# cmavro/GNN-RAG

Measured on AMD Instinct MI355X. Metric: kg_edges_aggregated_per_sec, higher is better.
Workload: dtype f32

## Files before the change

### gnn-rag_amd/csrc/dense_internal.h

```cpp
#pragma once
#include "gnnrag_common.h"

namespace gnnrag {

int tables_vq_launch_z(const gnnrag_csr* csr, const void* planes, const float* ins, const float* W, float* P, int32_t D,
                       int32_t I, int32_t only_dir, float* zero, int64_t zero_n, hipStream_t stream);

int update_b3_launch_z(const float* h, const float* nbr, const float* W, const float* b, const float* w_s,
                       const float* b_s, const float* mask, float* h_out, float* score, int64_t BN, int32_t D,
                       int32_t ldw, hipStream_t stream, bool score_zeroed);

int update_score_fused_rows(const float* h, const float* nbr, const uint8_t* add_flag, const float* W, const float* b,
                            const float* w_s, const float* b_s, const float* mask, float* h_out, float* score,
                            int64_t BN, int32_t D, int32_t I, int32_t math, hipStream_t stream, bool score_zeroed);
int update_b3_launch_f(const float* h, const float* nbr, const uint8_t* add_flag, const float* W, const float* b,
                       const float* w_s, const float* b_s, const float* mask, float* h_out, float* score, int64_t BN,
                       int32_t D, int32_t ldw, hipStream_t stream, bool score_zeroed);

bool update_rows_supported(const float* h, const float* nbr, const float* W, const float* h_out, int64_t BN, int32_t D,
                           int32_t I, int32_t math);
bool update_b3_shape_ok(int64_t BN, int32_t D, int32_t ldw);
int tables_small_launch(const gnnrag_csr* csr, const float* T_fwd, const float* T_inv, const float* ins, const float* W,
                        float* P, int32_t D, int32_t I, hipStream_t stream);

int frontier_build_z(const gnnrag_csr* csr, const float* dist, void* fws, size_t fws_bytes, float* zero_a,
                     int64_t zero_na, float* zero_b, int64_t zero_nb, hipStream_t stream);
const uint8_t* frontier_row_flags(const gnnrag_csr* csr, const void* fws);

int update_score_fused_z(const float* h, const float* nbr, const float* W, const float* b, const float* w_s,
                         const float* b_s, const float* mask, float* h_out, float* score, int64_t BN, int32_t D,
                         int32_t I, int32_t math, hipStream_t stream, bool score_zeroed);

bool rel_transform_accepts(const float* relfeat_fwd, const float* relfeat_inv, int64_t R1, int32_t D, int32_t L,
                           const gnnrag_layer_params* layers, int32_t pos_rows, const float* T_out, const void* planes_out);

}
```

### gnn-rag_amd/csrc/frontier.hip

```cpp
#include "dense_internal.h"

namespace gnnrag {

constexpr int kFrThreads = 1024;
constexpr int kFrSeedCap = 2048;
constexpr int kFrAltSeeds = 32;

struct FrontierWs {
  size_t counts, row_flag, rows, tflag, trows, seeds, seedinfo, total;
};

static FrontierWs frontier_ws(const gnnrag_csr* csr) {
  FrontierWs w;
  size_t off = 0;
  auto take = [&](size_t bytes) { size_t o = off; off = align_up(off + bytes, 256); return o; };
  const size_t BN = (size_t)csr->B * csr->N;
  const size_t RT = (size_t)(csr->rel_total > 0 ? csr->rel_total : 1);
  w.counts = take((size_t)2 * csr->B * sizeof(int32_t));
  w.row_flag = take(BN + 64);
  w.rows = take(BN * sizeof(int32_t));
  w.tflag = take(RT + 64);
  w.trows = take(RT * sizeof(int32_t));
  w.seeds = take((size_t)csr->B * kFrAltSeeds * sizeof(int32_t));
  w.seedinfo = take((size_t)2 * csr->B * sizeof(int32_t));
  w.total = off;
  return w;
}

__global__ __launch_bounds__(kFrThreads) void k_frontier_build(
    const float* __restrict__ dist, const int32_t* __restrict__ rp0, const int32_t* __restrict__ rp1,
    const int2* __restrict__ el0, const int2* __restrict__ el1, const int32_t* __restrict__ rel_off, int N,
    uint8_t* __restrict__ row_flag, int32_t* __restrict__ rows, uint8_t* __restrict__ tflag,
    int32_t* __restrict__ trows, int32_t* __restrict__ counts, int32_t* __restrict__ seeds,
    int32_t* __restrict__ seedinfo, float* __restrict__ zero_a, long long zero_na, float* __restrict__ zero_b,
    long long zero_nb) {
  __shared__ int s_seed[kFrSeedCap];
  __shared__ int s_ns, s_wsum[kFrThreads / 64];
  const int g = blockIdx.x, tid = threadIdx.x, lane = tid & 63, wave = tid >> 6;
  const int roff = rel_off[g], Rg = rel_off[g + 1] - roff;
  const size_t n0 = (size_t)g * N;
  for (long long i = (long long)blockIdx.x * kFrThreads + tid; i < zero_na; i += (long long)gridDim.x * kFrThreads) zero_a[i] = 0.f;
  for (long long i = (long long)blockIdx.x * kFrThreads + tid; i < zero_nb; i += (long long)gridDim.x * kFrThreads) zero_b[i] = 0.f;
  if (tid == 0) s_ns = 0;
  if (g == (int)gridDim.x - 1 && tid < 64) row_flag[(size_t)gridDim.x * N + tid] = 0;
  for (int i = tid; i < N; i += kFrThreads) row_flag[n0 + i] = 0;
  for (int i = tid; i < Rg; i += kFrThreads) tflag[roff + i] = 0;
  __syncthreads();
  for (int i = tid; i < N; i += kFrThreads) {
    if (dist[n0 + i] != 0.f) {
      const int k = atomicAdd(&s_ns, 1);
      if (k < kFrSeedCap) s_seed[k] = (int)n0 + i;
    }
  }
  __syncthreads();
  const int ns = s_ns;
  if (tid == 0) {
    int cnt = -1, facts = 0;
    if (ns <= kFrAltSeeds) {
      cnt = ns;
      for (int i = 1; i < ns; ++i) {
        const int v = s_seed[i];
        int j = i - 1;
        for (; j >= 0 && s_seed[j] > v; --j) s_seed[j + 1] = s_seed[j];
        s_seed[j + 1] = v;
      }
      for (int i = 0; i < ns; ++i) {
        const int sn = s_seed[i];
        seeds[g * kFrAltSeeds + i] = sn;
        facts += (rp0[sn + 1] - rp0[sn]) + (rp1[sn + 1] - rp1[sn]);
      }
    }
    seedinfo[2 * g] = cnt;
    seedinfo[2 * g + 1] = facts;
  }
  __syncthreads();
  if (ns > kFrSeedCap) {
    for (int i = tid; i < N; i += kFrThreads) row_flag[n0 + i] = 1;
    for (int i = tid; i < Rg; i += kFrThreads) tflag[roff + i] = 1;
  } else {
    for (int k = 0; k < ns; ++k) {
      const int s = s_seed[k];
#pragma unroll
      for (int dd = 0; dd < 2; ++dd) {
        const int32_t* rp = dd ? rp1 : rp0;
        const int2* el = dd ? el1 : el0;
        const int beg = rp[s], end = rp[s + 1];
        for (int j = beg + tid; j < end; j += kFrThreads) {
          const int2 e = el[j];
          row_flag[e.x] = 1;
          tflag[roff + e.y] = 1;
        }
      }
    }
  }
  __syncthreads();
  auto compact = [&](const uint8_t* flag, int n, int first, int32_t* list, int32_t* count_out) {
    int base = 0;
    for (int c0 = 0; c0 < n; c0 += kFrThreads) {
      const int i = c0 + tid;
      const bool on = i < n && flag[i] != 0;
      const unsigned long long m = __ballot(on);
      if (lane == 0) s_wsum[wave] = __popcll(m);
      __syncthreads();
      int off = base, tot = 0;
      for (int w = 0; w < kFrThreads / 64; ++w) {
        const int c = s_wsum[w];
        if (w < wave) off += c;
        tot += c;
      }
      if (on) list[off + __popcll(m & ((1ull << lane) - 1))] = first + i;
      base += tot;
      __syncthreads();
    }
    if (tid == 0) *count_out = base;
  };
  compact(row_flag + n0, N, (int)n0, rows + n0, counts + 2 * g);
  compact(tflag + roff, Rg, roff, trows + roff, counts + 2 * g + 1);
}

struct TabFrArgs {
  const float* T[2];
  const float* ins;
  const float* W;
  const int2* rel_rows;
  const int32_t* rel_off;
  const int32_t* list;
  const int32_t* counts;
  float* P;
  int32_t D, I, rel_total, B;
  int32_t dense;
};

__global__ __launch_bounds__(256) void k_tables_frontier(TabFrArgs a, int tiles_per_q) {
  __shared__ __attribute__((aligned(16))) float s_part[3][4][64][4];
  const int lane = threadIdx.x & 63, wave = threadIdx.x >> 6;
  const int fr = lane & 15, fg = lane >> 4;
  const int D = a.D, K = a.I * D, ldw = (2 * a.I + 1) * D;
  const int ncg = (D + 63) >> 6;
  const f32x4 zero4 = {0.f, 0.f, 0.f, 0.f};
  const int nitem = a.dense ? ((a.rel_total + 15) >> 4) * 2 * ncg : a.B * 2 * ncg;
  for (int item = blockIdx.x; item < nitem; item += gridDim.x)
  for (int tile = a.dense ? item / (2 * ncg) : 0; tile < (a.dense ? item / (2 * ncg) + 1 : tiles_per_q); ++tile) {
    int r = a.dense ? item % (2 * ncg) : item;
    const int cg = r % ncg; r /= ncg;
    const int d = r & 1; r >>= 1;
    const int g = a.dense ? 0 : r;
    const int cnt = a.dense ? a.rel_total : a.counts[2 * g + 1];
    if (tile * 16 >= cnt) break;
    const int32_t* list = a.dense ? nullptr : a.list + a.rel_off[g];
    const int c0 = cg * 64;
    const int m = tile * 16 + fr;
    const int prow = a.dense ? (m < cnt ? m : cnt - 1) : list[m < cnt ? m : cnt - 1];
    const int2 br = a.rel_rows[prow];
    const float* trow = a.T[d] + (size_t)br.y * D;
    const float* qrow = a.ins + (size_t)br.x * a.I * D;
    const float* wrow[4];
#pragma unroll
    for (int nt = 0; nt < 4; ++nt) wrow[nt] = a.W + (size_t)min(c0 + nt * 16 + fr, D - 1) * ldw + (size_t)(1 + d) * D;
    f32x4 acc[4] = {zero4, zero4, zero4, zero4};
    const int nkg = (K + 15) >> 4;
    for (int kg0 = wave; kg0 < nkg; kg0 += 16) {
      f32x4 av[4], bv[4][4];
#pragma unroll
      for (int u = 0; u < 4; ++u) {
        const int k = (kg0 + 4 * u) * 16 + fg * 4;
        av[u] = zero4;
#pragma unroll
        for (int nt = 0; nt < 4; ++nt) bv[u][nt] = zero4;
        if (k < K) {
          const int i = k / D, kk = k - i * D;
          const f32x4 t = *reinterpret_cast<const f32x4*>(trow + kk);
          const f32x4 q = *reinterpret_cast<const f32x4*>(qrow + (size_t)i * D + kk);
          av[u] = __builtin_elementwise_max(t * q, zero4);
#pragma unroll
          for (int nt = 0; nt < 4; ++nt) bv[u][nt] = *reinterpret_cast<const f32x4*>(wrow[nt] + (size_t)2 * i * D + kk);
        }
      }
#pragma unroll
      for (int u = 0; u < 4; ++u)
#pragma unroll
        for (int nt = 0; nt < 4; ++nt)
#pragma unroll
          for (int e = 0; e < 4; ++e) acc[nt] = __builtin_amdgcn_mfma_f32_16x16x4f32(av[u][e], bv[u][nt][e], acc[nt], 0, 0, 0);
    }
    if (wave > 0) {
#pragma unroll
      for (int nt = 0; nt < 4; ++nt) *reinterpret_cast<f32x4*>(&s_part[wave - 1][nt][lane][0]) = acc[nt];
    }
    __syncthreads();
    if (wave == 0) {
#pragma unroll
      for (int nt = 0; nt < 4; ++nt) {
        const f32x4 v = ((acc[nt] + *reinterpret_cast<const f32x4*>(&s_part[0][nt][lane][0])) +
                         *reinterpret_cast<const f32x4*>(&s_part[1][nt][lane][0])) +
                        *reinterpret_cast<const f32x4*>(&s_part[2][nt][lane][0]);
        const int col = c0 + nt * 16 + fr;
#pragma unroll
        for (int rr = 0; rr < 4; ++rr) {
          const int mm = tile * 16 + fg * 4 + rr;
          if (mm < cnt && col < D) a.P[((size_t)d * a.rel_total + (a.dense ? mm : list[mm])) * D + col] = v[rr];
        }
      }
    }
    __syncthreads();
  }
}

struct WalkFrArgs {
  const int32_t* rp0;
  const int32_t* rp1;
  const int2* edge_m;
  const int32_t* m_from;
  const float* w0;
  const float* w1;
  const float* dist;
  const float* P;
  const int32_t* rel_off;
  const int32_t* rows;
  const int32_t* counts;
  float* out;
  const int32_t* seeds;
  const int32_t* seedinfo;
  int64_t F;
  int32_t N, D, rel_total, B;
};

constexpr int kWfThreads = 256;
constexpr int kWfPer = 8;
constexpr int kWfCap = kWfThreads * kWfPer;
constexpr int kWfAltMin = 4096;

__global__ __launch_bounds__(kWfThreads) void k_walk_frontier(WalkFrArgs a, int per_q) {
  __shared__ int2 s_live[kWfCap];
  __shared__ int s_wsum[kWfPer * 4];
  __shared__ __attribute__((aligned(16))) float s_red[3][256];
  const int tid = threadIdx.x, lane = tid & 63, wave = tid >> 6;
  const int D = a.D;
  const int g = blockIdx.x / per_q;
  const int cnt = a.counts[2 * g];
  const int roff = a.rel_off[g], Rg = a.rel_off[g + 1] - roff;
  const int col = 4 * lane;
  const bool cok = col < D;
  const f32x4 zero4 = {0.f, 0.f, 0.f, 0.f};
  for (int it = blockIdx.x % per_q; it < cnt; it += per_q) {
    const int n = a.rows[(size_t)g * a.N + it];
    const int beg = a.rp0[n] + a.rp1[n], end = a.rp0[n + 1] + a.rp1[n + 1];
    f32x4 acc = zero4;
    bool split = false;
    const int nseed = a.seedinfo[2 * g];
    const bool alt = nseed > 0 && end - beg > kWfAltMin && a.seedinfo[2 * g + 1] <= ((end - beg) >> 2);
    if (alt && wave == 0) {
      for (int si = 0; si < nseed; ++si) {
        const int sn = a.seeds[g * kFrAltSeeds + si];
        const float ps = a.dist[sn];
        const int sb = a.rp0[sn] + a.rp1[sn], se = a.rp0[sn + 1] + a.rp1[sn + 1];
        for (int c0 = sb; c0 < se; c0 += 64) {
          const int j = c0 + lane;
          const int2 e = j < se ? a.edge_m[j] : make_int2(-1, 0);
          float p = 0.f;
          if (e.x == n) {
            p = ps;
            if (a.w0) {
              const int f = a.m_from[j];
              p *= f < a.F ? a.w0[f] : a.w1[f - a.F];
            }
          }
          unsigned long long m = __ballot(p != 0.f);
          while (m) {
            const int l = __builtin_ctzll(m);
            m &= m - 1;
            const float pl = __int_as_float(__builtin_amdgcn_readlane(__float_as_int(p), l));
            const int rm = __builtin_amdgcn_readlane(e.y, l);
            const int dq = rm > Rg ? 1 : 0;
            const int rl = dq ? rm - (Rg + 1) : rm;
            if (cok) acc += pl * *reinterpret_cast<const f32x4*>(a.P + ((size_t)(1 - dq) * a.rel_total + roff + rl) * D + col);
          }
        }
      }
    }
    for (int c0 = beg; c0 < (alt ? beg : end); c0 += kWfCap) {
      int2 e[kWfPer];
      float p[kWfPer];
#pragma unroll
      for (int u = 0; u < kWfPer; ++u) {
        const int j = c0 + u * kWfThreads + tid;
        e[u] = j < end ? a.edge_m[j] : make_int2(0, 0);
      }
#pragma unroll
      for (int u = 0; u < kWfPer; ++u) {
        const int j = c0 + u * kWfThreads + tid;
        p[u] = 0.f;
        if (j < end) {
          p[u] = a.dist[e[u].x];
          if (a.w0) {
            const int f = a.m_from[j];
            p[u] *= f < a.F ? a.w0[f] : a.w1[f - a.F];
          }
        }
      }
      unsigned long long mk[kWfPer];
#pragma unroll
      for (int u = 0; u < kWfPer; ++u) {
        mk[u] = __ballot(p[u] != 0.f);
        if (lane == 0) s_wsum[u * 4 + wave] = __popcll(mk[u]);
      }
      __syncthreads();
      int nl = 0;
#pragma unroll
      for (int u = 0; u < kWfPer; ++u) {
        int off = nl;
#pragma unroll
        for (int w = 0; w < 4; ++w) {
          const int t = s_wsum[u * 4 + w];
          if (w < wave) off += t;
          nl += t;
        }
        if (p[u] != 0.f) {
          const int rm = e[u].y;
          const int d = rm > Rg ? 1 : 0;
          const int rl = d ? rm - (Rg + 1) : rm;
          s_live[off + __popcll(mk[u] & ((1ull << lane) - 1))] = make_int2(__float_as_int(p[u]), d * a.rel_total + roff + rl);
        }
      }
      __syncthreads();
      if (nl <= 32 && !split) {
        if (wave == 0 && cok) {
          for (int k = 0; k < nl; ++k) {
            const int2 lv = s_live[k];
            const f32x4 t = *reinterpret_cast<const f32x4*>(a.P + (size_t)lv.y * D + col);
            acc += __int_as_float(lv.x) * t;
          }
        }
      } else {
        split = true;
        if (cok) {
          for (int k = wave; k < nl; k += 4) {
            const int2 lv = s_live[k];
            const f32x4 t = *reinterpret_cast<const f32x4*>(a.P + (size_t)lv.y * D + col);
            acc += __int_as_float(lv.x) * t;
          }
        }
      }
      __syncthreads();
    }
    if (split) {
      if (wave > 0) *reinterpret_cast<f32x4*>(&s_red[wave - 1][col]) = acc;
      __syncthreads();
      if (wave == 0)
        acc = ((acc + *reinterpret_cast<const f32x4*>(&s_red[0][col])) + *reinterpret_cast<const f32x4*>(&s_red[1][col])) +
              *reinterpret_cast<const f32x4*>(&s_red[2][col]);
      __syncthreads();
    }
    if (wave == 0 && cok) *reinterpret_cast<f32x4*>(a.out + (size_t)n * D + col) = acc;
  }
}

}

using namespace gnnrag;

extern "C" size_t gnnrag_frontier_workspace_bytes(const gnnrag_csr* csr) {
  if (!csr) return 0;
  return frontier_ws(csr).total;
}

extern "C" int gnnrag_frontier_supported(const gnnrag_csr* csr, int32_t D) {
  return csr && csr->edge_m && csr->m_from && D > 0 && D % 4 == 0 && D <= 256 ? 1 : 0;
}

int gnnrag::frontier_build_z(const gnnrag_csr* csr, const float* dist, void* fws, size_t fws_bytes, float* zero_a,
                             int64_t zero_na, float* zero_b, int64_t zero_nb, hipStream_t stream) {
  if (!csr || !dist || !fws) return GNNRAG_E_BADARG;
  const FrontierWs w = frontier_ws(csr);
  if (fws_bytes < w.total) return GNNRAG_E_WORKSPACE;
  char* base = (char*)fws;
  hipLaunchKernelGGL(k_frontier_build, dim3(csr->B), dim3(kFrThreads), 0, stream, dist, csr->row_ptr[0], csr->row_ptr[1],
                     (const int2*)csr->edge_l[0], (const int2*)csr->edge_l[1], csr->rel_off, csr->N,
                     (uint8_t*)(base + w.row_flag), (int32_t*)(base + w.rows), (uint8_t*)(base + w.tflag),
                     (int32_t*)(base + w.trows), (int32_t*)(base + w.counts), (int32_t*)(base + w.seeds),
                     (int32_t*)(base + w.seedinfo), zero_a, (long long)zero_na, zero_b,
                     (long long)zero_nb);
  GNNRAG_LAUNCH_CHECK();
  return 0;
}

extern "C" int gnnrag_frontier_build(const gnnrag_csr* csr, const float* dist, void* fws, size_t fws_bytes,
                                     gnnrag_stream_t stream) {
  return frontier_build_z(csr, dist, fws, fws_bytes, nullptr, 0, nullptr, 0, (hipStream_t)stream);
}

const uint8_t* gnnrag::frontier_row_flags(const gnnrag_csr* csr, const void* fws) {
  return (const uint8_t*)fws + frontier_ws(csr).row_flag;
}

static bool fr_aligned16(const void* a, const void* b = nullptr, const void* c = nullptr, const void* d = nullptr,
                         const void* e = nullptr) {
  return ((((uintptr_t)a | (uintptr_t)b | (uintptr_t)c | (uintptr_t)d | (uintptr_t)e) & 15) == 0);
}

extern "C" int gnnrag_relation_tables_frontier(const gnnrag_csr* csr, const void* fws, const float* T_fwd,
                                               const float* T_inv, const float* ins, const float* W, float* P,
                                               int32_t D, int32_t I, gnnrag_stream_t stream) {
  if (!csr || !fws || !T_fwd || !T_inv || !ins || !W || !P || I <= 0) return GNNRAG_E_BADARG;
  if (!gnnrag_frontier_supported(csr, D) || !fr_aligned16(T_fwd, T_inv, ins, W, P)) return GNNRAG_E_UNSUPPORTED;
  if (csr->rel_total == 0) return 0;
  const FrontierWs w = frontier_ws(csr);
  const char* base = (const char*)fws;
  TabFrArgs a;
  a.T[0] = T_fwd; a.T[1] = T_inv; a.ins = ins; a.W = W;
  a.rel_rows = (const int2*)csr->rel_rows;
  a.rel_off = csr->rel_off;
  a.list = (const int32_t*)(base + w.trows);
  a.counts = (const int32_t*)(base + w.counts);
  a.P = P; a.D = D; a.I = I; a.rel_total = csr->rel_total; a.B = csr->B; a.dense = 0;
  const int tiles_per_q = (csr->rel_max + 15) / 16;
  const int64_t nitem = (int64_t)csr->B * 2 * ((D + 63) / 64);
  hipLaunchKernelGGL(k_tables_frontier, dim3((unsigned)(nitem < 4096 ? nitem : 4096)), dim3(256), 0, (hipStream_t)stream, a,
                     tiles_per_q);
  GNNRAG_LAUNCH_CHECK();
  return 0;
}

extern "C" int gnnrag_aggregate_fused_frontier(const gnnrag_csr* csr, const void* fws, const float* dist,
                                               const float* P, float* out, int32_t D, gnnrag_stream_t stream) {
  if (!csr || !fws || !dist || !P || !out) return GNNRAG_E_BADARG;
  if (!gnnrag_frontier_supported(csr, D) || !fr_aligned16(P, out) || csr->N <= 0) return GNNRAG_E_UNSUPPORTED;
  const FrontierWs w = frontier_ws(csr);
  const char* base = (const char*)fws;
  WalkFrArgs a;
  a.rp0 = csr->row_ptr[0]; a.rp1 = csr->row_ptr[1];
  a.edge_m = (const int2*)csr->edge_m; a.m_from = csr->m_from;
  a.w0 = csr->w_gnn[0]; a.w1 = csr->w_gnn[1];
  a.dist = dist; a.P = P; a.rel_off = csr->rel_off;
  a.rows = (const int32_t*)(base + w.rows);
  a.counts = (const int32_t*)(base + w.counts);
  a.seeds = (const int32_t*)(base + w.seeds);
  a.seedinfo = (const int32_t*)(base + w.seedinfo);
  a.out = out; a.F = csr->F; a.N = csr->N; a.D = D; a.rel_total = csr->rel_total; a.B = csr->B;
  int per_q = 1024 / csr->B;
  if (per_q < 4) per_q = 4;
  if (per_q > 256) per_q = 256;
  if (per_q > csr->N) per_q = csr->N;
  hipLaunchKernelGGL(k_walk_frontier, dim3((unsigned)(csr->B * per_q)), dim3(kWfThreads), 0, (hipStream_t)stream, a, per_q);
  GNNRAG_LAUNCH_CHECK();
  return 0;
}

extern "C" int gnnrag_frontier_read(const gnnrag_csr* csr, const void* fws, int32_t* counts2, uint8_t* row_flag_host,
                                    gnnrag_stream_t stream) {
  if (!csr || !fws || !counts2) return GNNRAG_E_BADARG;
  const FrontierWs w = frontier_ws(csr);
  const char* base = (const char*)fws;
  int32_t* per_q = new int32_t[(size_t)2 * csr->B];
  hipError_t e = hipMemcpyAsync(per_q, base + w.counts, (size_t)2 * csr->B * sizeof(int32_t), hipMemcpyDeviceToHost,
                                (hipStream_t)stream);
  if (e == hipSuccess && row_flag_host)
    e = hipMemcpyAsync(row_flag_host, base + w.row_flag, (size_t)csr->B * csr->N, hipMemcpyDeviceToHost, (hipStream_t)stream);
  if (e == hipSuccess) e = hipStreamSynchronize((hipStream_t)stream);
  counts2[0] = counts2[1] = 0;
  for (int g = 0; g < csr->B; ++g) {
    counts2[0] += per_q[2 * g];
    counts2[1] += per_q[2 * g + 1];
  }
  delete[] per_q;
  return e == hipSuccess ? 0 : (int)e;
}

int gnnrag::tables_small_launch(const gnnrag_csr* csr, const float* T_fwd, const float* T_inv, const float* ins,
                                const float* W, float* P, int32_t D, int32_t I, hipStream_t stream) {
  if (D % 4 || D > 256 || csr->rel_total <= 0) return GNNRAG_E_UNSUPPORTED;
  if (2.0 * 2 * csr->rel_total * (double)I * D * D > 1.5e8) return GNNRAG_E_UNSUPPORTED;
  if ((((uintptr_t)T_fwd | (uintptr_t)T_inv | (uintptr_t)ins | (uintptr_t)W) & 15) != 0) return GNNRAG_E_UNSUPPORTED;
  TabFrArgs a;
  a.T[0] = T_fwd; a.T[1] = T_inv; a.ins = ins; a.W = W;
  a.rel_rows = (const int2*)csr->rel_rows;
  a.rel_off = csr->rel_off;
  a.list = nullptr; a.counts = nullptr;
  a.P = P; a.D = D; a.I = I; a.rel_total = csr->rel_total; a.B = csr->B; a.dense = 1;
  const int nitem = ((csr->rel_total + 15) / 16) * 2 * ((D + 63) / 64);
  hipLaunchKernelGGL(k_tables_frontier, dim3(nitem), dim3(256), 0, stream, a, 0);
  GNNRAG_LAUNCH_CHECK();
  return 0;
}
```

### gnn-rag_amd/csrc/softmax_layer.hip

```cpp
#include "gnnrag_common.h"
#include "dense_internal.h"

namespace gnnrag {

template <int ITEMS>
__global__ __launch_bounds__(1024) void k_masked_softmax(const float* __restrict__ score,
                                                         float* __restrict__ dist, int N) {
  __shared__ float red[16];
  __shared__ float bcast;
  const float* s = score + (size_t)blockIdx.x * N;
  float* o = dist + (size_t)blockIdx.x * N;
  const int lane = threadIdx.x & 63, wave = threadIdx.x >> 6;
  float v[ITEMS > 0 ? ITEMS : 1];

  float m = -INFINITY;
  if constexpr (ITEMS > 0) {
#pragma unroll
    for (int k = 0; k < ITEMS; ++k) {
      const int i = threadIdx.x + k * 1024;
      v[k] = i < N ? s[i] : -INFINITY;
      m = fmaxf(m, v[k]);
    }
  } else {
    for (int i = threadIdx.x; i < N; i += 1024) m = fmaxf(m, s[i]);
  }
#pragma unroll
  for (int off = 32; off > 0; off >>= 1) m = fmaxf(m, __shfl_xor(m, off, 64));
  if (lane == 0) red[wave] = m;
  __syncthreads();
  if (threadIdx.x == 0) {
    float mm = red[0];
    for (int w = 1; w < 16; ++w) mm = fmaxf(mm, red[w]);
    bcast = mm;
  }
  __syncthreads();
  m = bcast;
  __syncthreads();

  float sum = 0.f;
  if constexpr (ITEMS > 0) {
#pragma unroll
    for (int k = 0; k < ITEMS; ++k) {
      v[k] = expf(v[k] - m);
      sum += v[k];
    }
  } else {
    for (int i = threadIdx.x; i < N; i += 1024) sum += expf(s[i] - m);
  }
#pragma unroll
  for (int off = 32; off > 0; off >>= 1) sum += __shfl_xor(sum, off, 64);
  if (lane == 0) red[wave] = sum;
  __syncthreads();
  if (threadIdx.x == 0) {
    float t = 0.f;
    for (int w = 0; w < 16; ++w) t += red[w];
    bcast = t;
  }
  __syncthreads();
  const float total = bcast;
  if constexpr (ITEMS > 0) {
#pragma unroll
    for (int k = 0; k < ITEMS; ++k) {
      const int i = threadIdx.x + k * 1024;
      if (i < N) o[i] = v[k] / total;
    }
  } else {
    for (int i = threadIdx.x; i < N; i += 1024) o[i] = expf(s[i] - m) / total;
  }
}

template <int ITEMS>
__global__ __launch_bounds__(1024) void k_softmax_pairs(const float* __restrict__ score, float* __restrict__ dist, int N,
                                                        const int32_t* __restrict__ rp0, const int32_t* __restrict__ rp1,
                                                        const int2* __restrict__ em, const int32_t* __restrict__ from,
                                                        const float* __restrict__ w0, const float* __restrict__ w1,
                                                        int64_t F, int2* __restrict__ pr) {
  extern __shared__ float s_dist[];
  __shared__ float red[16];
  __shared__ float bcast;
  const int g = blockIdx.x, part = blockIdx.y, nparts = gridDim.y;
  const float* s = score + (size_t)g * N;
  float* o = dist + (size_t)g * N;
  const int lane = threadIdx.x & 63, wave = threadIdx.x >> 6;
  float v[ITEMS];
  float m = -INFINITY;
#pragma unroll
  for (int k = 0; k < ITEMS; ++k) {
    const int i = threadIdx.x + k * 1024;
    v[k] = i < N ? s[i] : -INFINITY;
    m = fmaxf(m, v[k]);
  }
#pragma unroll
  for (int off = 32; off > 0; off >>= 1) m = fmaxf(m, __shfl_xor(m, off, 64));
  if (lane == 0) red[wave] = m;
  __syncthreads();
  if (threadIdx.x == 0) {
    float mm = red[0];
    for (int w = 1; w < 16; ++w) mm = fmaxf(mm, red[w]);
    bcast = mm;
  }
  __syncthreads();
  m = bcast;
  __syncthreads();
  float sum = 0.f;
#pragma unroll
  for (int k = 0; k < ITEMS; ++k) {
    v[k] = expf(v[k] - m);
    sum += v[k];
  }
#pragma unroll
  for (int off = 32; off > 0; off >>= 1) sum += __shfl_xor(sum, off, 64);
  if (lane == 0) red[wave] = sum;
  __syncthreads();
  if (threadIdx.x == 0) {
    float t = 0.f;
    for (int w = 0; w < 16; ++w) t += red[w];
    bcast = t;
  }
  __syncthreads();
  const float total = bcast;
#pragma unroll
  for (int k = 0; k < ITEMS; ++k) {
    const int i = threadIdx.x + k * 1024;
    if (i < N) {
      const float d = v[k] / total;
      s_dist[i] = d;
      if (part == 0) o[i] = d;
    }
  }
  __syncthreads();
  const int64_t n0 = (int64_t)g * N;
  const int64_t beg = (int64_t)rp0[n0] + rp1[n0], end = (int64_t)rp0[n0 + N] + rp1[n0 + N];
  const int64_t lo = beg + (end - beg) * part / nparts, hi = beg + (end - beg) * (part + 1) / nparts;
  typedef int i32x2 __attribute__((ext_vector_type(2)));
  for (int64_t j = lo + threadIdx.x; j < hi; j += 1024) {
    const i32x2 e = __builtin_nontemporal_load(reinterpret_cast<const i32x2*>(em) + j);
    const unsigned s = (unsigned)(e.x - (int)n0);
    float p = s < (unsigned)N ? s_dist[s] : 0.f;
    if (w0) {
      const int f = from[j];
      p *= f < F ? w0[f] : w1[f - F];
    }
    pr[j] = make_int2(__float_as_int(p), e.y);
  }
}

__global__ __launch_bounds__(256) void k_stream_copy(const f32x4* __restrict__ src, f32x4* __restrict__ dst,
                                                     int64_t n4) {
  const int64_t stride = (int64_t)gridDim.x * 1024;
  for (int64_t base = (int64_t)blockIdx.x * 1024; base < n4; base += stride) {
    f32x4 v[4];
#pragma unroll
    for (int u = 0; u < 4; ++u) {
      const int64_t i = base + u * 256 + threadIdx.x;
      if (i < n4) v[u] = __builtin_nontemporal_load(src + i);
    }
#pragma unroll
    for (int u = 0; u < 4; ++u) {
      const int64_t i = base + u * 256 + threadIdx.x;
      if (i < n4) __builtin_nontemporal_store(v[u], dst + i);
    }
  }
}

struct LayerWs { size_t T_fwd, T_inv, planes, agg, P, nbr, partial, partial_bytes, fws, fws_bytes, total; };

static bool fused_is_cheaper(int64_t B, int64_t N, int64_t rel_total, int64_t D, int64_t I) {
  const double unfused = (double)B * N * (2 * I + 1) * D * D;
  const double fused = 2.0 * rel_total * I * D * D + (double)B * N * D * D;
  return fused < 0.8 * unfused;
}

static bool path_ok(int32_t path) {
  const int base = path & 0xf, flags = path & ~0xf & ~GNNRAG_PATH_SEED_PRIOR & ~GNNRAG_PATH_REUSE_PROJ;
  if (base < GNNRAG_PATH_AUTO || base > GNNRAG_PATH_FUSED) return false;
  return flags == 0 || flags == GNNRAG_PATH_ONLY_FWD || flags == GNNRAG_PATH_ONLY_INV;
}

static LayerWs layer_ws(const gnnrag_csr* csr, int32_t D, int32_t I) {
  LayerWs w;
  size_t off = 0;
  auto take = [&](size_t bytes) { size_t o = off; off = align_up(off + bytes, 256); return o; };
  const size_t BN = (size_t)csr->B * csr->N;
  w.T_fwd = take((size_t)2 * csr->R1 * D * sizeof(float));
  w.T_inv = w.T_fwd + (size_t)csr->R1 * D * sizeof(float);
  w.planes = take(tables_vq_shape_ok(D, I) ? tables_vq_planes_bytes(csr->R1) : 0);
  const size_t a_bytes = BN * 2 * I * D * sizeof(float);
  const size_t p_bytes = align_up((size_t)2 * (csr->rel_total > 0 ? csr->rel_total : 1) * D * sizeof(float), 256);
  const size_t n_bytes = (BN + 1) * D * sizeof(float);
  const size_t big = take(a_bytes > p_bytes + n_bytes ? a_bytes : p_bytes + n_bytes);
  w.agg = big;
  w.P = big;
  w.nbr = big + p_bytes;
  w.partial_bytes = gnnrag_aggregate_workspace_bytes(csr, D, I);
  w.partial = take(w.partial_bytes);
  w.fws_bytes = gnnrag_frontier_workspace_bytes(csr);
  w.fws = take(w.fws_bytes);
  w.total = off;
  return w;
}

static bool planes_wanted(const gnnrag_csr* csr, int32_t D, int32_t I, int32_t path, int32_t math) {
  const bool fused = (path & 0xf) == GNNRAG_PATH_FUSED ||
                     ((path & 0xf) == GNNRAG_PATH_AUTO && fused_is_cheaper(csr->B, csr->N, csr->rel_total, D, I));
  return fused && math != GNNRAG_MATH_FP32 && tables_vq_shape_ok(D, I) && csr->rel_total >= 1024;
}

}

using namespace gnnrag;

extern "C" int gnnrag_masked_softmax(const float* score, float* dist, int32_t B, int32_t N,
                                     gnnrag_stream_t stream) {
  if (!score || !dist || B <= 0 || N <= 0) return GNNRAG_E_BADARG;
  if (N <= 2048) hipLaunchKernelGGL(k_masked_softmax<2>, dim3(B), dim3(1024), 0, (hipStream_t)stream, score, dist, N);
  else if (N <= 8192) hipLaunchKernelGGL(k_masked_softmax<8>, dim3(B), dim3(1024), 0, (hipStream_t)stream, score, dist, N);
  else hipLaunchKernelGGL(k_masked_softmax<0>, dim3(B), dim3(1024), 0, (hipStream_t)stream, score, dist, N);
  GNNRAG_LAUNCH_CHECK();
  return 0;
}

extern "C" int gnnrag_stream_copy(const float* src, float* dst, int64_t n, gnnrag_stream_t stream) {
  if (!src || !dst || n < 0 || (n & 3)) return GNNRAG_E_BADARG;
  if (n == 0) return 0;
  hipLaunchKernelGGL(k_stream_copy, dim3(256 * 16), dim3(256), 0, (hipStream_t)stream, (const f32x4*)src,
                     (f32x4*)dst, n / 4);
  GNNRAG_LAUNCH_CHECK();
  return 0;
}

extern "C" size_t gnnrag_layer_workspace_bytes(const gnnrag_csr* csr, int32_t D, int32_t I) {
  if (!csr || D <= 0 || I <= 0) return 0;
  return layer_ws(csr, D, I).total;
}

static int finish_softmax(const gnnrag_csr* csr, const LayerWs& w, char* base, const float* score, float* dist_out, int32_t D,
                          bool want_pairs, bool* pairs_done, gnnrag_stream_t stream) {
  if (pairs_done) *pairs_done = false;
  const char* env = getenv("GNNRAG_SOFTMAX_PAIRS");
  const bool enabled = !(env && env[0] == '0');
  if (want_pairs && pairs_done && enabled && csr->N <= 8192 && csr->edge_m) {
    PriorPairsTarget t;
    const int rc = prior_pairs_target(csr, D, base + w.partial, w.partial_bytes, &t);
    if (rc) return rc;
    if (t.ok) {
      int parts = (512 + csr->B - 1) / csr->B;
      parts = parts < 1 ? 1 : parts > 8 ? 8 : parts;
      const size_t lds = (size_t)csr->N * sizeof(float);
      if (csr->N <= 2048)
        hipLaunchKernelGGL(k_softmax_pairs<2>, dim3(csr->B, parts), dim3(1024), lds, (hipStream_t)stream, score, dist_out,
                           csr->N, csr->row_ptr[0], csr->row_ptr[1], t.edge_m, t.m_from, t.w0, t.w1, t.F, t.pairs);
      else
        hipLaunchKernelGGL(k_softmax_pairs<8>, dim3(csr->B, parts), dim3(1024), lds, (hipStream_t)stream, score, dist_out,
                           csr->N, csr->row_ptr[0], csr->row_ptr[1], t.edge_m, t.m_from, t.w0, t.w1, t.F, t.pairs);
      GNNRAG_LAUNCH_CHECK();
      *pairs_done = true;
      return 0;
    }
  }
  return gnnrag_masked_softmax(score, dist_out, csr->B, csr->N, stream);
}

static int layer_body(const gnnrag_csr* csr, const LayerWs& w, char* base, const float* h, const float* dist,
                      const float* ins, const float* T_fwd, const float* T_inv, const void* planes, const float* W_e2e,
                      const float* b_e2e, const float* w_score, const float* b_score, const float* mask,
                      float* h_out, float* score_out, float* dist_out, int32_t D, int32_t I, int32_t path,
                      int32_t math, gnnrag_stream_t stream, bool pairs_ready = false, bool* pairs_for_next = nullptr) {
  if (pairs_for_next) *pairs_for_next = false;
  const int64_t BN = (int64_t)csr->B * csr->N;
  int rc;
  const int only = (path & GNNRAG_PATH_ONLY_FWD) ? 0 : (path & GNNRAG_PATH_ONLY_INV) ? 1 : -1;
  const bool seed_prior = (path & GNNRAG_PATH_SEED_PRIOR) != 0;
  path &= 0xf;
  if (path == GNNRAG_PATH_AUTO)
    path = fused_is_cheaper(csr->B, csr->N, csr->rel_total, D, I) ? GNNRAG_PATH_FUSED : GNNRAG_PATH_UNFUSED;
  if (path == GNNRAG_PATH_FUSED) {
    float* P = (float*)(base + w.P);
    float* nbr = (float*)(base + w.nbr);
    const bool one_dir = only >= 0 && gnnrag_aggregate_fused_variant(csr, D) != GNNRAG_WALK_L2_GATHER;
    const bool fr_aligned = ((((uintptr_t)ins | (uintptr_t)W_e2e | (uintptr_t)T_fwd | (uintptr_t)T_inv | (uintptr_t)P |
                               (uintptr_t)nbr | (uintptr_t)dist) & 15) == 0) && csr->N > 0;
    const bool frontier_form = seed_prior && only < 0 && fr_aligned && gnnrag_frontier_supported(csr, D) && csr->rel_total > 0;
    if (frontier_form) {
      void* fws = base + w.fws;
      const bool gated = update_rows_supported(h, nbr, W_e2e, h_out, BN, D, I, math);
      if (!gated) GNNRAG_HIP(hipMemsetAsync(nbr, 0, (size_t)BN * D * sizeof(float), (hipStream_t)stream));
      rc = frontier_build_z(csr, dist, fws, w.fws_bytes, score_out, BN, nbr + (size_t)BN * D, D, (hipStream_t)stream);
      if (rc) return rc;
      rc = gnnrag_relation_tables_frontier(csr, fws, T_fwd, T_inv, ins, W_e2e, P, D, I, stream);
      if (rc) return rc;
      rc = gnnrag_aggregate_fused_frontier(csr, fws, dist, P, nbr, D, stream);
      if (rc) return rc;
      rc = update_score_fused_rows(h, nbr, gated ? frontier_row_flags(csr, fws) : nullptr, W_e2e, b_e2e, w_score, b_score,
                                   mask, h_out, score_out, BN, D, I, math, (hipStream_t)stream, true);
      if (rc) return rc;
      return finish_softmax(csr, w, base, score_out, dist_out, D, only < 0, pairs_for_next, stream);
    }
    rc = GNNRAG_E_UNSUPPORTED;
    bool score_zeroed = false;
    if (planes && math != GNNRAG_MATH_FP32 && csr->rel_total > 0) {
      rc = tables_vq_launch_z(csr, planes, ins, W_e2e, P, D, I, one_dir ? only : -1, score_out, BN, (hipStream_t)stream);
      score_zeroed = rc == 0;
    }
    if (rc == GNNRAG_E_UNSUPPORTED) rc = gnnrag_relation_tables(csr, T_fwd, T_inv, ins, W_e2e, P, D, I, math, stream);
    if (rc) return rc;
    rc = aggregate_fused_dirs(csr, dist, P, nbr, D, one_dir ? 2 - only : 0, base + w.partial, w.partial_bytes,
                              (hipStream_t)stream, pairs_ready && !one_dir);
    if (rc) return rc;
    rc = update_score_fused_z(h, nbr, W_e2e, b_e2e, w_score, b_score, mask, h_out, score_out, BN, D, I, math,
                              (hipStream_t)stream, score_zeroed);
    if (rc) return rc;
    return finish_softmax(csr, w, base, score_out, dist_out, D, only < 0, pairs_for_next, stream);
  } else {
    float* agg = (float*)(base + w.agg);
    rc = gnnrag_aggregate(csr, dist, ins, T_fwd, T_inv, agg, D, I, base + w.partial, w.partial_bytes, stream);
    if (rc) return rc;
    rc = gnnrag_update_score(h, agg, W_e2e, b_e2e, w_score, b_score, mask, h_out, score_out, BN, D, I, math,
                             stream);
    if (rc) return rc;
  }
  return gnnrag_masked_softmax(score_out, dist_out, csr->B, csr->N, stream);
}

static int rel_projections(const gnnrag_csr* csr, int32_t n, const gnnrag_layer_params* layers,
                           const float* relfeat_fwd, const float* relfeat_inv, int32_t pos_rows, float* T,
                           void* planes, bool* planes_written, int32_t D, int32_t math, gnnrag_stream_t stream) {
  *planes_written = false;
  if ((D & 3) == 0) {
    const int rc = gnnrag_rel_transform(relfeat_fwd, relfeat_inv, csr->R1, D, n, layers, pos_rows, T, planes, stream);
    if (rc == 0) *planes_written = planes != nullptr;
    if (rc != GNNRAG_E_UNSUPPORTED) return rc;
  }
  const size_t RD = (size_t)csr->R1 * D;
  for (int j = 0; j < n; ++j) {
    const gnnrag_layer_params& p = layers[j];
    const int rc = gnnrag_linear_pair(relfeat_fwd, relfeat_inv, csr->R1, D, p.W_rel, p.b_rel, p.pos_fwd, p.pos_inv,
                                      p.pos_fwd ? pos_rows : 0, T + 2 * j * RD, T + (2 * j + 1) * RD, D, math, stream);
    if (rc) return rc;
  }
  return 0;
}

extern "C" size_t gnnrag_stack_workspace_bytes(const gnnrag_csr* csr, int32_t L, int32_t D, int32_t I) {
  if (!csr || L <= 0 || D <= 0 || I <= 0) return 0;
  return layer_ws(csr, D, I).total + align_up((size_t)L * 2 * csr->R1 * D * sizeof(float), 256) +
         align_up(tables_vq_shape_ok(D, I) ? (size_t)L * tables_vq_planes_bytes(csr->R1) : 0, 256);
}

extern "C" int gnnrag_reason_layer(const gnnrag_csr* csr, const float* h, const float* dist, const float* ins,
                                   const float* relfeat_fwd, const float* relfeat_inv, const float* W_rel,
                                   const float* b_rel, const float* pos_fwd, const float* pos_inv,
                                   int32_t pos_rows, const float* W_e2e, const float* b_e2e,
                                   const float* w_score, const float* b_score, const float* mask,
                                   float* h_out, float* score_out, float* dist_out, void* workspace,
                                   size_t workspace_bytes, int32_t D, int32_t I, int32_t path, int32_t math,
                                   gnnrag_stream_t stream) {
  if (!csr || !h || !dist || !ins || !relfeat_fwd || !relfeat_inv || !W_rel || !b_rel || !W_e2e || !b_e2e ||
      !w_score || !b_score || !mask || !h_out || !score_out || !dist_out || !workspace || D <= 0 || I <= 0)
    return GNNRAG_E_BADARG;
  if (!path_ok(path)) return GNNRAG_E_BADARG;
  const LayerWs w = layer_ws(csr, D, I);
  if (workspace_bytes < w.total) return GNNRAG_E_WORKSPACE;
  char* base = (char*)workspace;
  float* T_fwd = (float*)(base + w.T_fwd);
  float* T_inv = (float*)(base + w.T_inv);
  const gnnrag_layer_params p = {W_rel, b_rel, pos_fwd, pos_inv, W_e2e, b_e2e};
  void* planes = planes_wanted(csr, D, I, path, math) ? (void*)(base + w.planes) : nullptr;
  bool planes_written = false;
  const int rc = rel_projections(csr, 1, &p, relfeat_fwd, relfeat_inv, pos_rows, T_fwd, planes, &planes_written, D, math,
                                 stream);
  if (rc) return rc;
  if (!planes_written) planes = nullptr;
  return layer_body(csr, w, base, h, dist, ins, T_fwd, T_inv, planes, W_e2e, b_e2e, w_score, b_score, mask, h_out, score_out,
                    dist_out, D, I, path, math, stream);
}

extern "C" int gnnrag_reason_stack(const gnnrag_csr* csr, int32_t L, const gnnrag_layer_params* layers,
                                   const float* h0, const float* dist0, const float* ins,
                                   const float* relfeat_fwd, const float* relfeat_inv, int32_t pos_rows,
                                   const float* w_score, const float* b_score, const float* mask, float* h_out,
                                   float* score_out, float* dist_out, void* workspace, size_t workspace_bytes,
                                   int32_t D, int32_t I, int32_t path, int32_t math, gnnrag_stream_t stream) {
  if (!csr || L <= 0 || !layers || !h0 || !dist0 || !ins || !relfeat_fwd || !relfeat_inv || !w_score || !b_score ||
      !mask || !h_out || !score_out || !dist_out || !workspace || D <= 0 || I <= 0)
    return GNNRAG_E_BADARG;
  if (!path_ok(path)) return GNNRAG_E_BADARG;
  for (int j = 0; j < L; ++j)
    if (!layers[j].W_rel || !layers[j].b_rel || !layers[j].W_e2e || !layers[j].b_e2e) return GNNRAG_E_BADARG;
  const LayerWs w = layer_ws(csr, D, I);
  if (workspace_bytes < w.total) return GNNRAG_E_WORKSPACE;
  char* base = (char*)workspace;
  const size_t BN = (size_t)csr->B * csr->N;
  const size_t RD = (size_t)csr->R1 * D;
  const bool upfront = L > 1 && workspace_bytes >= gnnrag_stack_workspace_bytes(csr, L, D, I);
  float* T0 = (float*)(base + w.T_fwd);
  float* Tall = (float*)(base + w.total);
  const bool want_planes = planes_wanted(csr, D, I, path, math);
  const size_t plane_bytes = tables_vq_planes_bytes(csr->R1);
  char* planes_all = base + w.total + align_up((size_t)L * 2 * RD * sizeof(float), 256);
  bool planes_written = false;
  const bool reuse = upfront && (path & GNNRAG_PATH_REUSE_PROJ) != 0;
  path &= ~GNNRAG_PATH_REUSE_PROJ;
  if (reuse) {
    planes_written = want_planes && rel_transform_accepts(relfeat_fwd, relfeat_inv, csr->R1, D, L, layers, pos_rows, Tall,
                                                          planes_all);
  } else if (upfront) {
    const int rc = rel_projections(csr, L, layers, relfeat_fwd, relfeat_inv, pos_rows, Tall,
                                   want_planes ? planes_all : nullptr, &planes_written, D, math, stream);
    if (rc) return rc;
  }
  const float* h = h0;
  const float* dist = dist0;
  bool pairs_ready = false;
  for (int j = 0; j < L; ++j) {
    const gnnrag_layer_params& p = layers[j];
    float* hj = h_out + (size_t)j * BN * D;
    float* sj = score_out + (size_t)j * BN;
    float* dj = dist_out + (size_t)j * BN;
    float* T = upfront ? Tall + (size_t)j * 2 * RD : T0;
    void* planes = !want_planes ? nullptr : upfront ? (void*)(planes_all + (size_t)j * plane_bytes) : (void*)(base + w.planes);
    if (!upfront) {
      const int rc = rel_projections(csr, 1, &p, relfeat_fwd, relfeat_inv, pos_rows, T, planes, &planes_written, D, math,
                                     stream);
      if (rc) return rc;
    }
    if (!planes_written) planes = nullptr;
    bool pairs_next = false;
    const int rc = layer_body(csr, w, base, h, dist, ins, T, T + RD, planes, p.W_e2e, p.b_e2e, w_score, b_score, mask, hj, sj,
                              dj, D, I, j == 0 ? path : (path & ~GNNRAG_PATH_SEED_PRIOR), math, stream, pairs_ready,
                              j + 1 < L ? &pairs_next : nullptr);
    if (rc) return rc;
    pairs_ready = pairs_next;
    h = hj;
    dist = dj;
  }
  return 0;
}

struct gnnrag_graph {
  hipGraph_t graph;
  hipGraphExec_t exec;
};

extern "C" int gnnrag_reason_stack_capture(const gnnrag_csr* csr, int32_t L, const gnnrag_layer_params* layers,
                                           const float* h0, const float* dist0, const float* ins,
                                           const float* relfeat_fwd, const float* relfeat_inv, int32_t pos_rows,
                                           const float* w_score, const float* b_score, const float* mask,
                                           float* h_out, float* score_out, float* dist_out, void* workspace,
                                           size_t workspace_bytes, int32_t D, int32_t I, int32_t path, int32_t math,
                                           gnnrag_stream_t stream_, gnnrag_graph** out) {
  if (!out) return GNNRAG_E_BADARG;
  *out = nullptr;
  hipStream_t stream = (hipStream_t)stream_;
  GNNRAG_HIP(hipStreamBeginCapture(stream, hipStreamCaptureModeThreadLocal));
  const int rc = gnnrag_reason_stack(csr, L, layers, h0, dist0, ins, relfeat_fwd, relfeat_inv, pos_rows, w_score,
                                     b_score, mask, h_out, score_out, dist_out, workspace, workspace_bytes, D, I, path,
                                     math, stream);
  hipGraph_t graph = nullptr;
  const hipError_t e = hipStreamEndCapture(stream, &graph);
  if (rc) {
    if (graph) (void)hipGraphDestroy(graph);
    return rc;
  }
  if (e != hipSuccess) return (int)e;
  hipGraphExec_t exec = nullptr;
  const hipError_t e2 = hipGraphInstantiate(&exec, graph, nullptr, nullptr, 0);
  if (e2 != hipSuccess) {
    (void)hipGraphDestroy(graph);
    return (int)e2;
  }
  gnnrag_graph* g = new gnnrag_graph{graph, exec};
  *out = g;
  return 0;
}

extern "C" int gnnrag_graph_launch(gnnrag_graph* graph, gnnrag_stream_t stream) {
  if (!graph) return GNNRAG_E_BADARG;
  GNNRAG_HIP(hipGraphLaunch(graph->exec, (hipStream_t)stream));
  return 0;
}

extern "C" int gnnrag_graph_destroy(gnnrag_graph* graph) {
  if (!graph) return 0;
  (void)hipGraphExecDestroy(graph->exec);
  (void)hipGraphDestroy(graph->graph);
  delete graph;
  return 0;
}

extern "C" int gnnrag_abi_version(void) { return GNNRAG_ABI_VERSION; }

extern "C" const char* gnnrag_error_string(int code) {
  switch (code) {
    case 0: return "success";
    case GNNRAG_E_BADARG: return "gnnrag: bad argument (null pointer, negative or inconsistent size)";
    case GNNRAG_E_UNSUPPORTED: return "gnnrag: shape outside the compiled kernel set";
    case GNNRAG_E_WORKSPACE: return "gnnrag: caller-provided buffer too small";
    case GNNRAG_E_TUPLE:
      return "gnnrag: edge tuple out of range: node ids must lie in [0, B*N), relation ids in [0, R1), and a fact "
             "may not connect two questions";
  }
  if (code > 0) return hipGetErrorString((hipError_t)code);
  return "gnnrag: unknown error";
}
```

### gnn-rag_amd/csrc/tables_b3.hip

```cpp
#include "gnnrag_common.h"
#include "dense_internal.h"

namespace gnnrag {

#ifndef GNNRAG_TAB_TPW
#define GNNRAG_TAB_TPW 3
#endif
#ifndef GNNRAG_TAB_MINBLK
#define GNNRAG_TAB_MINBLK 2
#endif
constexpr int kTabTPW = GNNRAG_TAB_TPW;
constexpr int kTabNTH = 7;
constexpr int kTabNKB = 7;
constexpr int kTabSlots = 26;
constexpr int kTabQBytes = 160 * 1024 - 3 * kTabNTH * 16 * kTabSlots * 16 - 64;

struct TabArgs {
  const float* T[2];
  const float* ins;
  const float* W;
  float* P;
  const int2* rows;
  int32_t M, D, I, ldw;
  int32_t ct0;
  int32_t npass;
};

__device__ __forceinline__ int opaque_i(int x) {
  asm volatile("" : "+v"(x));
  return x;
}

template <int CTRL, int BANK>
__device__ __forceinline__ float dpp_b3(float old, float x) {
  return __int_as_float(__builtin_amdgcn_update_dpp(__float_as_int(old), __float_as_int(x), CTRL, 0xf, BANK, false));
}
__device__ __forceinline__ float row16_sum4_b3(const float (&v)[4], int lane) {
  const bool b0 = lane & 1, b1 = lane & 2;
  float w2[2];
#pragma unroll
  for (int j = 0; j < 2; ++j) {
    const float send = b0 ? v[j] : v[j + 2];
    w2[j] = (b0 ? v[j + 2] : v[j]) + dpp_b3<0xB1, 0xf>(send, send);
  }
  const float send = b1 ? w2[0] : w2[1];
  float w = (b1 ? w2[1] : w2[0]) + dpp_b3<0x4E, 0xf>(send, send);
  const float t4 = dpp_b3<0x104, 0x5>(w, w);
  w += dpp_b3<0x114, 0xA>(t4, w);
  w += dpp_b3<0x128, 0xf>(w, w);
  return w;
}

__device__ __forceinline__ int tab_lds_row(int j) {
  if (j < 64) return ((j & 3) << 4) + (j >> 2);
  return j;
}

__device__ __forceinline__ constexpr int tab_stage_rows(int ctn) { return ctn < kTabNTH ? ctn * 16 + 1 : ctn * 16; }

template <int CTN, bool QLDS>
__device__ __forceinline__ void tables_b3_part(const TabArgs& a, unsigned char* lds, int col0, int bmin, int nq) {
  constexpr int RB = kTabSlots * 16;
  constexpr int PL = kTabNTH * 16 * RB;
  constexpr int ctn = CTN;
  const int tid = threadIdx.x, lane = tid & 63, wave = tid >> 6;
  const int fr = lane & 15, fg = lane >> 4;
  const int d = blockIdx.y;
  const int D = a.D, I = a.I;
  const int ncol = min(ctn * 16, D - col0);
  const float* T = a.T[d];
  float* P = a.P + (size_t)d * a.M * D;
  const f32x4 zero4 = {0.f, 0.f, 0.f, 0.f};
  constexpr int NKB = kTabNKB;
  const int KC = D >> 2;

  const long long U = ((long long)a.M + 15) >> 4;
  const int c0 = (int)(U * blockIdx.x / gridDim.x), c1 = (int)(U * (blockIdx.x + 1) / gridDim.x);
  const int nchunk = c1 - c0;
  const int w0 = c0 + (int)((long long)nchunk * wave / 8), w1 = c0 + (int)((long long)nchunk * (wave + 1) / 8);

  if (tid < 16) reinterpret_cast<unsigned*>(lds + 3 * PL)[tid] = 0u;
  float* qarea = reinterpret_cast<float*>(lds + 3 * PL + 64);
  constexpr bool q_in_lds = QLDS;
  if (q_in_lds) {
    const float* src = a.ins + (size_t)bmin * I * D;
    for (int x = tid * 4; x < nq * I * D; x += 512 * 4)
      *reinterpret_cast<f32x4*>(qarea + x) = *reinterpret_cast<const f32x4*>(src + x);
  }

  for (int pass = 0; pass < a.npass; ++pass) {
    const int tbase = w0 + pass * kTabTPW;
    const int ntile = max(0, min(kTabTPW, w1 - tbase));
    f32x4 acc[kTabTPW][CTN];
#pragma unroll
    for (int j = 0; j < kTabTPW; ++j)
#pragma unroll
      for (int nt = 0; nt < CTN; ++nt) acc[j][nt] = zero4;

    for (int i = 0; i < I; ++i) {
      __syncthreads();
      {
        const int wcol = (1 + 2 * i + d) * D;
        const int total = tab_stage_rows(ctn) * kTabSlots * 2;
        constexpr int UN = 6;
        for (int base = 0; base < total; base += 512 * UN) {
          f32x4 v[UN];
          int off[UN];
#pragma unroll
          for (int u = 0; u < UN; ++u) {
            const int idx = base + u * 512 + tid;
            const int j = idx / (kTabSlots * 2), kc = idx - j * (kTabSlots * 2);
            v[u] = zero4;
            off[u] = idx < total ? tab_lds_row(j) * RB + kc * 8 : -1;
            if (idx < total && j < ncol && kc < KC)
              v[u] = *reinterpret_cast<const f32x4*>(a.W + (size_t)(col0 + j) * a.ldw + wcol + 4 * kc);
          }
#pragma unroll
          for (int u = 0; u < UN; ++u) {
            if (off[u] >= 0) {
              const Split3 sp = split3(v[u]);
              unsigned char* dst = lds + off[u];
              *reinterpret_cast<uint2*>(dst) = sp.hi;
              *reinterpret_cast<uint2*>(dst + PL) = sp.mid;
              *reinterpret_cast<uint2*>(dst + 2 * PL) = sp.lo;
            }
          }
        }
      }
      __syncthreads();

      int toff[kTabTPW], qoff[kTabTPW];
#pragma unroll
      for (int j = 0; j < kTabTPW; ++j) {
        const int m = min((tbase + (j < ntile ? j : 0)) * 16 + fr, a.M - 1);
        const int2 br = a.rows[m];
        toff[j] = br.y * D + 8 * fg;
        qoff[j] = ((br.x - bmin) * I + i) * D + 8 * fg;
      }
      const int kmax = D - 8;
      f32x4 traw[kTabTPW][2];
#pragma unroll
      for (int j = 0; j < kTabTPW; ++j) {
        const float* tp = T + toff[j] + (min(8 * fg, kmax) - 8 * fg);
        traw[j][0] = *reinterpret_cast<const f32x4*>(tp);
        traw[j][1] = *reinterpret_cast<const f32x4*>(tp + 4);
      }
      for (int kb = 0; kb < NKB; ++kb) {
        const bool kok = 32 * kb + 8 * fg <= kmax;
        const int kbn = min(kb + 1, NKB - 1);
        const int kon = min(32 * kbn + 8 * fg, kmax) - 8 * fg;
        const int koq = min(32 * kb + 8 * fg, kmax) - 8 * fg;
        const unsigned char* wb = lds + fr * RB + kb * 64 + fg * 16;
#pragma unroll
        for (int j = 0; j < kTabTPW; ++j) {
          if (j < ntile) {
            const f32x4 t0 = traw[j][0], t1 = traw[j][1];
            {
              const float* tp = T + toff[j] + kon;
              traw[j][0] = *reinterpret_cast<const f32x4*>(tp);
              traw[j][1] = *reinterpret_cast<const f32x4*>(tp + 4);
            }
            __builtin_amdgcn_sched_barrier(0);
            f32x4 q0, q1;
            if constexpr (QLDS) {
              const float* qp = qarea + qoff[j] + koq;
              q0 = *reinterpret_cast<const f32x4*>(qp);
              q1 = *reinterpret_cast<const f32x4*>(qp + 4);
            } else {
              const float* qp = a.ins + (size_t)bmin * I * D + qoff[j] + koq;
              q0 = *reinterpret_cast<const f32x4*>(qp);
              q1 = *reinterpret_cast<const f32x4*>(qp + 4);
            }
            const Split3 s0 = split3(kok ? __builtin_elementwise_max(t0 * q0, zero4) : zero4);
            const Split3 s1 = split3(kok ? __builtin_elementwise_max(t1 * q1, zero4) : zero4);
            typedef unsigned u32x4 __attribute__((ext_vector_type(4)));
            bf16x8 ap[3];
            ap[0] = __builtin_bit_cast(bf16x8, (u32x4){s0.hi.x, s0.hi.y, s1.hi.x, s1.hi.y});
            ap[1] = __builtin_bit_cast(bf16x8, (u32x4){s0.mid.x, s0.mid.y, s1.mid.x, s1.mid.y});
            ap[2] = __builtin_bit_cast(bf16x8, (u32x4){s0.lo.x, s0.lo.y, s1.lo.x, s1.lo.y});
            constexpr int PA[6] = {1, 2, 0, 1, 0, 0};
            constexpr int PB[6] = {1, 0, 2, 0, 1, 0};
#pragma unroll
            for (int nt = 0; nt < CTN; nt += 2) {
              bf16x8 b0[3], b1[3];
#pragma unroll
              for (int pl = 0; pl < 3; ++pl) {
                b0[pl] = __builtin_bit_cast(bf16x8, *reinterpret_cast<const f32x4*>(wb + pl * PL + nt * 16 * RB));
                b1[pl] = b0[pl];
                if (nt + 1 < CTN)
                  b1[pl] = __builtin_bit_cast(bf16x8, *reinterpret_cast<const f32x4*>(wb + pl * PL + (nt + 1) * 16 * RB));
              }
#pragma unroll
              for (int p = 0; p < 6; ++p) {
                acc[j][nt] = __builtin_amdgcn_mfma_f32_16x16x32_bf16(ap[PA[p]], b0[PB[p]], acc[j][nt], 0, 0, 0);
                if (nt + 1 < CTN)
                  acc[j][nt + 1] = __builtin_amdgcn_mfma_f32_16x16x32_bf16(ap[PA[p]], b1[PB[p]], acc[j][nt + 1], 0, 0, 0);
              }
            }
          }
        }
      }
    }

#pragma unroll
    for (int j = 0; j < kTabTPW; ++j) {
      if (j < ntile) {
        const int rbase = (tbase + j) * 16 + 4 * fg;
#pragma unroll
        for (int q = 0; q < 4; ++q) {
          const int row = rbase + q;
          if (row < a.M) {
            float* prow = P + (size_t)row * D + col0;
            static_assert(CTN >= 4, "a column part holds at least the interleaved group");
            {
              const f32x4 v = {acc[j][0][q], acc[j][1][q], acc[j][2][q], acc[j][3][q]};
              const int c = 4 * fr;
              if (c + 4 <= ncol) *reinterpret_cast<f32x4*>(prow + c) = v;
              else {
#pragma unroll
                for (int e = 0; e < 4; ++e)
                  if (c + e < ncol) prow[c + e] = v[e];
              }
            }
#pragma unroll
            for (int nt = 4; nt < CTN; ++nt) {
              const int c = nt * 16 + fr;
              if (c < ncol) prow[c] = acc[j][nt][q];
            }
          }
        }
      }
    }
  }
}

__global__ __launch_bounds__(512, GNNRAG_TAB_MINBLK) void k_tables_b3(TabArgs a) {
  extern __shared__ __attribute__((aligned(16))) unsigned char lds[];
  const int NT = (a.D + 15) >> 4;
  const int h = blockIdx.z;
  const int ctn = h == 0 ? a.ct0 : NT - a.ct0;
  const int col0 = h == 0 ? 0 : a.ct0 * 16;
  const long long U = ((long long)a.M + 15) >> 4;
  const int c0 = (int)(U * blockIdx.x / gridDim.x), c1 = (int)(U * (blockIdx.x + 1) / gridDim.x);
  const int rlo = min(c0 * 16, a.M - 1), rhi = min(c1 * 16, a.M) - 1;
  const int bmin = a.rows[rlo].x, bmax = a.rows[max(rhi, rlo)].x;
  const int nq = bmax - bmin + 1;
  const bool q_in_lds = (size_t)nq * a.I * a.D * sizeof(float) <= kTabQBytes;
#define GNNRAG_TAB_CASE(N)                                                  \
  case N:                                                                   \
    if (q_in_lds) tables_b3_part<N, true>(a, lds, col0, bmin, nq);          \
    else tables_b3_part<N, false>(a, lds, col0, bmin, nq);                  \
    break;
  switch (ctn) {
    GNNRAG_TAB_CASE(6) GNNRAG_TAB_CASE(7)
    default: break;
  }
#undef GNNRAG_TAB_CASE
}

constexpr int kVqHalf = 32 * kTabNKB;
constexpr int kVqRowB = 2 * kVqHalf * 2;
#ifndef GNNRAG_VQ_TPW
#define GNNRAG_VQ_TPW 5
#endif
#ifndef GNNRAG_VQ_UN
#define GNNRAG_VQ_UN 3
#endif
constexpr int kVqTPW = GNNRAG_VQ_TPW;

struct VqArgs {
  const unsigned char* planes;
  const float* ins;
  const float* W;
  float* P;
  const int2* rows;
  const int* rel_off;
  int32_t M, D, I, ldw, R1;
  int32_t ct0;
  int32_t nchunk;
  int32_t dir0;
  float* zero;
  int64_t zero_n;
};

template <int CTN, int UN>
__device__ __forceinline__ void vq_stage(const VqArgs& a, unsigned char* lds, const float* qarea, int col0, int ncol,
                                         int d, int s) {
  constexpr int RB = kTabSlots * 16;
  constexpr int PL = kTabNTH * 16 * RB;
  const int tid = threadIdx.x;
  const int D = a.D, I = a.I, KC = D >> 2;
  const f32x4 zero4 = {0.f, 0.f, 0.f, 0.f};
  const int total = tab_stage_rows(CTN) * kTabSlots * 2;
  for (int base = 0; base < total; base += 512 * UN) {
    f32x4 v[UN];
#pragma unroll
    for (int u = 0; u < UN; ++u) v[u] = zero4;
    for (int i = 0; i < I; ++i) {
      f32x4 w[UN];
      const float* wsrc = a.W + (size_t)col0 * a.ldw + (1 + 2 * i + d) * D;
#pragma unroll
      for (int u = 0; u < UN; ++u) {
        const int idx = base + u * 512 + tid;
        const int j = idx / (kTabSlots * 2), kc = idx - j * (kTabSlots * 2);
        w[u] = *reinterpret_cast<const f32x4*>(wsrc + (size_t)min(j, ncol - 1) * a.ldw + 4 * min(kc, KC - 1));
      }
#pragma unroll
      for (int u = 0; u < UN; ++u) {
        const int idx = base + u * 512 + tid;
        const int kc = idx % (kTabSlots * 2);
        f32x4 q = *reinterpret_cast<const f32x4*>(qarea + i * D + 4 * min(kc, KC - 1));
        q = __builtin_elementwise_max(s ? -q : q, zero4);
        v[u] += w[u] * q;
      }
    }
#pragma unroll
    for (int u = 0; u < UN; ++u) {
      const int idx = base + u * 512 + tid;
      const int j = idx / (kTabSlots * 2), kc = idx - j * (kTabSlots * 2);
      if (idx < total) {
        const Split3 sp = split3(j < ncol && kc < KC ? v[u] : zero4);
        unsigned char* dst = lds + tab_lds_row(j) * RB + kc * 8;
        *reinterpret_cast<uint2*>(dst) = sp.hi;
        *reinterpret_cast<uint2*>(dst + PL) = sp.mid;
        *reinterpret_cast<uint2*>(dst + 2 * PL) = sp.lo;
      }
    }
  }
}

template <int CTN>
__device__ __forceinline__ void tables_vq_part(const VqArgs& a, unsigned char* lds, int col0) {
  constexpr int RB = kTabSlots * 16;
  constexpr int PL = kTabNTH * 16 * RB;
  constexpr int NKB = kTabNKB;
  const int tid = threadIdx.x, lane = tid & 63, wave = tid >> 6;
  const int fr = lane & 15, fg = lane >> 4;
  const int d = a.dir0 + blockIdx.y;
  const int g = blockIdx.x / a.nchunk, ch = blockIdx.x - g * a.nchunk;
  const int D = a.D, I = a.I;
  const int r0 = a.rel_off[g], r1 = a.rel_off[g + 1];
  if (r1 <= r0) return;
  const int ncol = min(CTN * 16, D - col0);
  const int KC = D >> 2;
  const f32x4 zero4 = {0.f, 0.f, 0.f, 0.f};
  float* P = a.P + (size_t)d * a.M * D;
  const unsigned char* planes = a.planes + (size_t)d * 3 * a.R1 * kVqRowB;
  const size_t plane_stride = (size_t)a.R1 * kVqRowB;

  const int U = (r1 - r0 + 15) >> 4;
  const int c0 = U * ch / a.nchunk, c1 = U * (ch + 1) / a.nchunk;
  const int wv = __builtin_amdgcn_readfirstlane(wave);
  const int w0 = c0 + (c1 - c0) * wv / 8, w1 = c0 + (c1 - c0) * (wv + 1) / 8;
  const int npass = ((c1 - c0 + 7) / 8 + kVqTPW - 1) / kVqTPW;

  if (tid < 16) reinterpret_cast<unsigned*>(lds + 3 * PL)[tid] = 0u;
  float* qarea = reinterpret_cast<float*>(lds + 3 * PL + 64);
  for (int x = tid * 4; x < I * D; x += 512 * 4)
    *reinterpret_cast<f32x4*>(qarea + x) = *reinterpret_cast<const f32x4*>(a.ins + (size_t)g * I * D + x);

  for (int pass = 0; pass < npass; ++pass) {
    const int tbase = w0 + pass * kVqTPW;
    const int ntile = max(0, min(kVqTPW, w1 - tbase));
    f32x4 acc[kVqTPW][CTN];
#pragma unroll
    for (int j = 0; j < kVqTPW; ++j)
#pragma unroll
      for (int nt = 0; nt < CTN; ++nt) acc[j][nt] = zero4;
    unsigned aoff[kVqTPW];
#pragma unroll
    for (int j = 0; j < kVqTPW; ++j) {
      const int m = min(r0 + (tbase + (j < ntile ? j : 0)) * 16 + fr, r1 - 1);
      aoff[j] = (unsigned)a.rows[m].y * (unsigned)kVqRowB + (unsigned)fg * 16u;
    }
    const unsigned char* const plane_base[3] = {planes, planes + plane_stride, planes + 2 * plane_stride};

    for (int s = 0; s < 2; ++s) {
      __syncthreads();
      vq_stage<CTN, GNNRAG_VQ_UN>(a, lds, qarea, col0, ncol, d, s);
      __syncthreads();

      bf16x8 ap[kVqTPW][3];
#pragma unroll
      for (int j = 0; j < kVqTPW; ++j)
#pragma unroll
        for (int pl = 0; pl < 3; ++pl)
          ap[j][pl] = __builtin_bit_cast(bf16x8, *reinterpret_cast<const f32x4*>(plane_base[pl] + (aoff[j] + (unsigned)(s * (kVqHalf * 2)))));
      for (int kb = 0; kb < NKB; ++kb) {
        const int kbn = min(kb + 1, NKB - 1);
        const unsigned char* wb = lds + fr * RB + kb * 64 + fg * 16;
        constexpr int PA[6] = {1, 2, 0, 1, 0, 0};
        constexpr int PB[6] = {1, 0, 2, 0, 1, 0};
#pragma unroll
        for (int j = 0; j < kVqTPW; ++j) {
          if (j < ntile) {
#pragma unroll
            for (int nt = 0; nt < CTN; nt += 2) {
              bf16x8 b0[3], b1[3];
#pragma unroll
              for (int pl = 0; pl < 3; ++pl) {
                b0[pl] = __builtin_bit_cast(bf16x8, *reinterpret_cast<const f32x4*>(wb + pl * PL + nt * 16 * RB));
                b1[pl] = b0[pl];
                if (nt + 1 < CTN)
                  b1[pl] = __builtin_bit_cast(bf16x8, *reinterpret_cast<const f32x4*>(wb + pl * PL + (nt + 1) * 16 * RB));
              }
#pragma unroll
              for (int p = 0; p < 6; ++p) {
                acc[j][nt] = __builtin_amdgcn_mfma_f32_16x16x32_bf16(ap[j][PA[p]], b0[PB[p]], acc[j][nt], 0, 0, 0);
                if (nt + 1 < CTN)
                  acc[j][nt + 1] = __builtin_amdgcn_mfma_f32_16x16x32_bf16(ap[j][PA[p]], b1[PB[p]], acc[j][nt + 1], 0, 0, 0);
              }
            }
          }
#pragma unroll
          for (int pl = 0; pl < 3; ++pl)
            ap[j][pl] = __builtin_bit_cast(bf16x8, *reinterpret_cast<const f32x4*>(plane_base[pl] + (aoff[j] + (unsigned)(s * (kVqHalf * 2) + kbn * 64))));
        }
      }
    }

#pragma unroll
    for (int j = 0; j < kVqTPW; ++j) {
      if (j < ntile) {
        const int rbase = r0 + (tbase + j) * 16 + 4 * fg;
#pragma unroll
        for (int q = 0; q < 4; ++q) {
          const int row = rbase + q;
          if (row < r1) {
            float* prow = P + (size_t)row * D + col0;
            static_assert(CTN >= 4, "a column part holds at least the interleaved group");
            {
              const f32x4 v = {acc[j][0][q], acc[j][1][q], acc[j][2][q], acc[j][3][q]};
              const int c = 4 * fr;
              if (c + 4 <= ncol) *reinterpret_cast<f32x4*>(prow + c) = v;
              else {
#pragma unroll
                for (int e = 0; e < 4; ++e)
                  if (c + e < ncol) prow[c + e] = v[e];
              }
            }
#pragma unroll
            for (int nt = 4; nt < CTN; ++nt) {
              const int c = nt * 16 + fr;
              if (c < ncol) prow[c] = acc[j][nt][q];
            }
          }
        }
      }
    }
  }
}

__global__ __launch_bounds__(512, 2) void k_tables_vq(VqArgs a) {
  extern __shared__ __attribute__((aligned(16))) unsigned char lds[];
  if (a.zero) {
    const int64_t nb = (int64_t)gridDim.x * gridDim.y * gridDim.z;
    const int64_t lin = blockIdx.x + (int64_t)gridDim.x * (blockIdx.y + (int64_t)gridDim.y * blockIdx.z);
    for (int64_t i = lin * 512 + threadIdx.x; i < a.zero_n; i += nb * 512) a.zero[i] = 0.f;
  }
  const int NT = (a.D + 15) >> 4;
  const int h = blockIdx.z;
  const int ctn = h == 0 ? a.ct0 : NT - a.ct0;
  const int col0 = h == 0 ? 0 : a.ct0 * 16;
  switch (ctn) {
    case 6: tables_vq_part<6>(a, lds, col0); break;
    case 7: tables_vq_part<7>(a, lds, col0); break;
    default: break;
  }
}

struct UpdB3Args {
  const float* A;
  const float* W;
  const float* bias;
  const float* add;
  const float* w_s;
  const float* b_s;
  const float* mask;
  float* C;
  float* score;
  const uint8_t* add_flag;
  int32_t M, D, ldw, ct0;
};

template <int CTN, bool FL>
__device__ __forceinline__ void update_b3_part(const UpdB3Args& a, unsigned char* lds, int col0, bool first_part,
                                               int chunk, int nchunks) {
  constexpr int RB = kTabSlots * 16;
  constexpr int PL = kTabNTH * 16 * RB;
  constexpr int NKB = kTabNKB;
  const int tid = threadIdx.x, lane = tid & 63, wave = tid >> 6;
  const int fr = lane & 15, fg = lane >> 4;
  const int D = a.D;
  const int ncol = min(CTN * 16, D - col0);
  const int KC = D >> 2;
  const f32x4 zero4 = {0.f, 0.f, 0.f, 0.f};
  float* Bl = reinterpret_cast<float*>(lds + 3 * PL + 64);
  float* Sl = Bl + kTabNTH * 16;

  if (tid < 16) reinterpret_cast<unsigned*>(lds + 3 * PL)[tid] = 0u;
  for (int j = tid; j < kTabNTH * 16; j += 512) {
    Bl[j] = (j < ncol && a.bias) ? a.bias[col0 + j] : 0.f;
    Sl[j] = j < ncol ? a.w_s[col0 + j] : 0.f;
  }
  {
    const int total = tab_stage_rows(CTN) * kTabSlots * 2;
    constexpr int UN = 6;
    for (int base = 0; base < total; base += 512 * UN) {
      f32x4 v[UN];
      int off[UN];
#pragma unroll
      for (int u = 0; u < UN; ++u) {
        const int idx = base + u * 512 + tid;
        const int j = idx / (kTabSlots * 2), kc = idx - j * (kTabSlots * 2);
        v[u] = zero4;
        off[u] = idx < total ? tab_lds_row(j) * RB + kc * 8 : -1;
        if (idx < total && j < ncol && kc < KC)
          v[u] = *reinterpret_cast<const f32x4*>(a.W + (size_t)(col0 + j) * a.ldw + 4 * kc);
      }
#pragma unroll
      for (int u = 0; u < UN; ++u) {
        if (off[u] >= 0) {
          const Split3 sp = split3(v[u]);
          unsigned char* dst = lds + off[u];
          *reinterpret_cast<uint2*>(dst) = sp.hi;
          *reinterpret_cast<uint2*>(dst + PL) = sp.mid;
          *reinterpret_cast<uint2*>(dst + 2 * PL) = sp.lo;
        }
      }
    }
  }
  const long long U = ((long long)a.M + 15) >> 4;
  const int c0 = (int)(U * chunk / nchunks), c1 = (int)(U * (chunk + 1) / nchunks);
  const int nch = c1 - c0;
  int t = c0 + (int)((long long)nch * wave / 8);
  const int tend = c0 + (int)((long long)nch * (wave + 1) / 8);
  const int kmax = D - 8;
  const unsigned char* Ab = reinterpret_cast<const unsigned char*>(a.A);
  const unsigned char* addb = reinterpret_cast<const unsigned char*>(a.add);
  unsigned char* Cb = reinterpret_cast<unsigned char*>(a.C);
  const unsigned rowB = (unsigned)D * 4u;
  const unsigned k6B = (unsigned)min(32 * (NKB - 1) + 8 * fg, kmax) * 4u;
  auto a_rowoff = [&](int tile) -> unsigned { return (unsigned)min(tile * 16 + fr, a.M - 1) * rowB; };
  auto a_piece = [&](unsigned rowoff, int kb, int half) -> f32x4 {
    const unsigned off = kb < NKB - 1 ? rowoff + 32u * (unsigned)fg + (unsigned)(128 * kb + 16 * half)
                                      : rowoff + k6B + (unsigned)(16 * half);
    return *reinterpret_cast<const f32x4*>(Ab + off);
  };
  f32x4 ra[NKB][2];
  if (t < tend) {
    const unsigned ro = a_rowoff(t);
#pragma unroll
    for (int kb = 0; kb < NKB; ++kb) {
      ra[kb][0] = a_piece(ro, kb, 0);
      ra[kb][1] = a_piece(ro, kb, 1);
    }
  }
  const float bs = a.b_s[0];
  const unsigned cgB = (unsigned)(col0 + min(4 * fr, ncol - 4)) * 4u;
  unsigned ctB[CTN > 4 ? CTN - 4 : 1];
#pragma unroll
  for (int nt = 4; nt < CTN; ++nt) ctB[nt - 4] = (unsigned)(col0 + min(nt * 16 + fr, ncol - 1)) * 4u;
  unsigned fl_next = 0x01010101u;
  if (FL && t < tend) fl_next = *reinterpret_cast<const unsigned*>(a.add_flag + (size_t)t * 16 + 4 * fg);
  __syncthreads();

  for (; t < tend; ++t) {
    const int rbase = t * 16 + 4 * fg;
    const unsigned fl = fl_next;
    if (FL) fl_next = *reinterpret_cast<const unsigned*>(a.add_flag + (size_t)(t + 1 < tend ? t + 1 : t) * 16 + 4 * fg);
    f32x4 addg[4];
    float addt[CTN > 4 ? CTN - 4 : 1][4];
#pragma unroll
    for (int q = 0; q < 4; ++q) {
      int row = min(rbase + q, a.M - 1);
      if (FL && ((fl >> (8 * q)) & 0xffu) == 0u) row = a.M;
      const unsigned ro = (unsigned)row * rowB;
      addg[q] = *reinterpret_cast<const f32x4*>(addb + (ro + cgB));
#pragma unroll
      for (int nt = 4; nt < CTN; ++nt) addt[nt - 4][q] = *reinterpret_cast<const float*>(addb + (ro + ctB[nt - 4]));
    }
    float mrow = 0.f;
    {
      const int srow = min(rbase + (2 * (fr & 1) + ((fr >> 1) & 1)), a.M - 1);
      mrow = a.mask[srow];
    }
    __builtin_amdgcn_sched_barrier(0);
    f32x4 acc[CTN];
#pragma unroll
    for (int nt = 0; nt < CTN; ++nt) acc[nt] = zero4;
    const unsigned ro_next = a_rowoff(t + 1 < tend ? t + 1 : t);
    const unsigned char* wbp[3];
#pragma unroll
    for (int pl = 0; pl < 3; ++pl) {
      unsigned o = (unsigned)(fr * RB + fg * 16 + pl * PL);
      asm volatile("" : "+v"(o));
      wbp[pl] = lds + o;
    }
    constexpr int PA[6] = {1, 2, 0, 1, 0, 0};
    constexpr int PB[6] = {1, 0, 2, 0, 1, 0};
#pragma unroll
    for (int kb = 0; kb < NKB; ++kb) {
      typedef unsigned u32x4 __attribute__((ext_vector_type(4)));
      bf16x8 ap[3];
      const bool kok = kb < NKB - 1 || 32 * kb + 8 * fg <= kmax;
      const Split3 s0 = split3(kok ? ra[kb][0] : zero4);
      const Split3 s1 = split3(kok ? ra[kb][1] : zero4);
      ap[0] = __builtin_bit_cast(bf16x8, (u32x4){s0.hi.x, s0.hi.y, s1.hi.x, s1.hi.y});
      ap[1] = __builtin_bit_cast(bf16x8, (u32x4){s0.mid.x, s0.mid.y, s1.mid.x, s1.mid.y});
      ap[2] = __builtin_bit_cast(bf16x8, (u32x4){s0.lo.x, s0.lo.y, s1.lo.x, s1.lo.y});
      ra[kb][0] = a_piece(ro_next, kb, 0);
      ra[kb][1] = a_piece(ro_next, kb, 1);
#pragma unroll
      for (int nt = 0; nt < CTN; nt += 2) {
        bf16x8 b0[3], b1[3];
#pragma unroll
        for (int pl = 0; pl < 3; ++pl) {
          b0[pl] = __builtin_bit_cast(bf16x8, *reinterpret_cast<const f32x4*>(wbp[pl] + (nt * 16 * RB + kb * 64)));
          b1[pl] = b0[pl];
          if (nt + 1 < CTN)
            b1[pl] = __builtin_bit_cast(bf16x8, *reinterpret_cast<const f32x4*>(wbp[pl] + ((nt + 1) * 16 * RB + kb * 64)));
        }
#pragma unroll
        for (int p = 0; p < 6; ++p) {
          acc[nt] = __builtin_amdgcn_mfma_f32_16x16x32_bf16(ap[PA[p]], b0[PB[p]], acc[nt], 0, 0, 0);
          if (nt + 1 < CTN)
            acc[nt + 1] = __builtin_amdgcn_mfma_f32_16x16x32_bf16(ap[PA[p]], b1[PB[p]], acc[nt + 1], 0, 0, 0);
        }
      }
    }
    float part[4] = {0.f, 0.f, 0.f, 0.f};
    const f32x4 bias_g = *reinterpret_cast<const f32x4*>(Bl + min(4 * fr, kTabNTH * 16 - 4));
    const f32x4 ws_g = *reinterpret_cast<const f32x4*>(Sl + min(4 * fr, kTabNTH * 16 - 4));
#pragma unroll
    for (int q = 0; q < 4; ++q) {
      const int row = rbase + q;
      const unsigned ro = (unsigned)min(row, a.M - 1) * rowB;
      f32x4 v = {acc[0][q], acc[1][q], acc[2][q], acc[3][q]};
      v = __builtin_elementwise_max((v + bias_g) + addg[q], zero4);
      const int c = 4 * fr;
      if (c + 4 > ncol) {
        v = zero4;
      } else if (row < a.M) {
        *reinterpret_cast<f32x4*>(Cb + (ro + cgB)) = v;
      }
      part[q] += v[0] * ws_g[0] + v[1] * ws_g[1] + v[2] * ws_g[2] + v[3] * ws_g[3];
#pragma unroll
      for (int nt = 4; nt < CTN; ++nt) {
        const int cc = nt * 16 + fr;
        float x = fmaxf((acc[nt][q] + Bl[cc]) + addt[nt - 4][q], 0.f);
        if (cc >= ncol) x = 0.f;
        else if (row < a.M) *reinterpret_cast<float*>(Cb + (ro + ctB[nt - 4])) = x;
        part[q] += x * Sl[cc];
      }
    }
    {
      const float tot = row16_sum4_b3(part, lane);
      const int srow = rbase + (2 * (fr & 1) + ((fr >> 1) & 1));
      if (fr < 4 && srow < a.M) {
        const float share = first_part ? (tot + bs) + (1.0f - mrow) * kVeryNeg : tot;
        atomicAdd(a.score + srow, share);
      }
    }
  }
}

template <bool FL>
__global__ __launch_bounds__(512, 2) void k_update_b3(UpdB3Args a, int nchunks) {
  extern __shared__ __attribute__((aligned(16))) unsigned char lds[];
  const int blk = blockIdx.x;
  const int NT = (a.D + 15) >> 4;
  const int h = (blk >> 3) & 1;
  const int chunk = (blk >> 4) * 8 + (blk & 7);
  if (chunk >= nchunks) return;
  if (h == 0) update_b3_part<kTabNTH, FL>(a, lds, 0, true, chunk, nchunks);
  else if (NT - a.ct0 == 6) update_b3_part<6, FL>(a, lds, a.ct0 * 16, false, chunk, nchunks);
}

int update_b3_launch(const float* h, const float* nbr, const float* W, const float* b, const float* w_s, const float* b_s,
                     const float* mask, float* h_out, float* score, int64_t BN, int32_t D, int32_t ldw,
                     hipStream_t stream) {
  return update_b3_launch_z(h, nbr, W, b, w_s, b_s, mask, h_out, score, BN, D, ldw, stream, false);
}

int update_b3_launch_z(const float* h, const float* nbr, const float* W, const float* b, const float* w_s,
                       const float* b_s, const float* mask, float* h_out, float* score, int64_t BN, int32_t D,
                       int32_t ldw, hipStream_t stream, bool score_zeroed) {
  return update_b3_launch_f(h, nbr, nullptr, W, b, w_s, b_s, mask, h_out, score, BN, D, ldw, stream, score_zeroed);
}

bool update_b3_shape_ok(int64_t BN, int32_t D, int32_t ldw) {
  return !(D % 8 || (D + 31) / 32 != kTabNKB || (D + 15) / 16 != 13 || BN < 8192 || (BN + 1) * D * 4 >= ((int64_t)1 << 32) || ldw % 4);
}

int update_b3_launch_f(const float* h, const float* nbr, const uint8_t* add_flag, const float* W, const float* b,
                       const float* w_s, const float* b_s, const float* mask, float* h_out, float* score, int64_t BN,
                       int32_t D, int32_t ldw, hipStream_t stream, bool score_zeroed) {
  if (!update_b3_shape_ok(BN, D, ldw)) return GNNRAG_E_UNSUPPORTED;
  if ((((uintptr_t)h | (uintptr_t)nbr | (uintptr_t)W | (uintptr_t)h_out) & 15) != 0) return GNNRAG_E_UNSUPPORTED;
  UpdB3Args a;
  memset(&a, 0, sizeof(a));
  a.A = h; a.W = W; a.bias = b; a.add = nbr; a.w_s = w_s; a.b_s = b_s; a.mask = mask; a.C = h_out; a.score = score;
  a.M = (int32_t)BN; a.D = D; a.ldw = ldw; a.ct0 = kTabNTH;
  a.add_flag = add_flag;
  if (add_flag && ((uintptr_t)add_flag & 3)) return GNNRAG_E_UNSUPPORTED;
  int cus = 0;
  {
    const int rc = device_cu_count(&cus);
    if (rc) return rc;
  }
  const long long U = (BN + 15) / 16;
  int chunks = cus / 2;
  if (chunks < 1) chunks = 1;
  if ((long long)chunks * 8 > U) chunks = (int)((U + 7) / 8);
  if (!score_zeroed) GNNRAG_HIP(hipMemsetAsync(score, 0, (size_t)BN * sizeof(float), stream));
  static DeviceMask cap, cap_f;
  {
    const int rc = add_flag ? raise_lds_cap(k_update_b3<true>, cap_f) : raise_lds_cap(k_update_b3<false>, cap);
    if (rc) return rc;
  }
  const int nblk = ((chunks + 7) / 8) * 16;
  if (add_flag) hipLaunchKernelGGL(k_update_b3<true>, dim3(nblk), dim3(512), 160 * 1024, stream, a, chunks);
  else hipLaunchKernelGGL(k_update_b3<false>, dim3(nblk), dim3(512), 160 * 1024, stream, a, chunks);
  GNNRAG_LAUNCH_CHECK();
  return 0;
}

size_t tables_vq_planes_bytes(int64_t R1) { return (size_t)2 * 3 * R1 * kVqRowB; }

bool tables_vq_shape_ok(int32_t D, int32_t I) {
  return D % 8 == 0 && (D + 31) / 32 == kTabNKB && (D + 15) / 16 == 13 && I >= 1 &&
         (size_t)I * D * sizeof(float) <= (size_t)kTabQBytes;
}

int tables_vq_launch(const gnnrag_csr* csr, const void* planes, const float* ins, const float* W, float* P, int32_t D,
                     int32_t I, int32_t only_dir, hipStream_t stream) {
  return tables_vq_launch_z(csr, planes, ins, W, P, D, I, only_dir, nullptr, 0, stream);
}

int tables_vq_launch_z(const gnnrag_csr* csr, const void* planes, const float* ins, const float* W, float* P, int32_t D,
                       int32_t I, int32_t only_dir, float* zero, int64_t zero_n, hipStream_t stream) {
  if (!tables_vq_shape_ok(D, I) || csr->rel_total < 1024 || only_dir > 1) return GNNRAG_E_UNSUPPORTED;
  if ((((uintptr_t)planes | (uintptr_t)ins | (uintptr_t)W | (uintptr_t)P) & 15) != 0) return GNNRAG_E_UNSUPPORTED;
  VqArgs a;
  memset(&a, 0, sizeof(a));
  a.planes = (const unsigned char*)planes; a.ins = ins; a.W = W; a.P = P;
  a.rows = (const int2*)csr->rel_rows; a.rel_off = csr->rel_off;
  a.M = csr->rel_total; a.D = D; a.I = I; a.ldw = (2 * I + 1) * D; a.R1 = csr->R1;
  const int NT = (D + 15) / 16;
  a.ct0 = (NT + 1) / 2;
  int cus = 0;
  {
    const int rc = device_cu_count(&cus);
    if (rc) return rc;
  }
  const int ndir = only_dir < 0 ? 2 : 1;
  a.dir0 = only_dir < 0 ? 0 : only_dir;
  int nchunk = cus / (csr->B * 2 * ndir);
  const int tiles_max = (csr->rel_max + 15) / 16;
  if (nchunk > tiles_max / 8) nchunk = tiles_max / 8;
  if (nchunk < 1) nchunk = 1;
  a.nchunk = nchunk;
  a.zero = zero;
  a.zero_n = zero ? zero_n : 0;
  static DeviceMask cap;
  {
    const int rc = raise_lds_cap(k_tables_vq, cap);
    if (rc) return rc;
  }
  hipLaunchKernelGGL(k_tables_vq, dim3(csr->B * nchunk, ndir, 2), dim3(512), 160 * 1024, stream, a);
  GNNRAG_LAUNCH_CHECK();
  return 0;
}

int tables_b3_launch(const gnnrag_csr* csr, const float* T_fwd, const float* T_inv, const float* ins, const float* W,
                     float* P, int32_t D, int32_t I, hipStream_t stream) {
  if (D % 8 || (D + 31) / 32 != kTabNKB || (D + 15) / 16 != 13 || csr->rel_total < 1024) return GNNRAG_E_UNSUPPORTED;
  if ((((uintptr_t)T_fwd | (uintptr_t)T_inv | (uintptr_t)ins | (uintptr_t)W | (uintptr_t)P) & 15) != 0)
    return GNNRAG_E_UNSUPPORTED;
  TabArgs a;
  memset(&a, 0, sizeof(a));
  a.T[0] = T_fwd; a.T[1] = T_inv; a.ins = ins; a.W = W; a.P = P;
  a.rows = (const int2*)csr->rel_rows;
  a.M = csr->rel_total; a.D = D; a.I = I; a.ldw = (2 * I + 1) * D;
  const int NT = (D + 15) / 16;
  a.ct0 = NT <= kTabNTH ? NT : (NT + 1) / 2;
  const int parts = NT <= kTabNTH ? 1 : 2;
  int cus = 0;
  {
    const int rc = device_cu_count(&cus);
    if (rc) return rc;
  }
  const long long U = ((long long)a.M + 15) / 16;
  int chunks = cus / (2 * parts);
  if (chunks < 1) chunks = 1;
  if ((long long)chunks * 8 > U) chunks = (int)((U + 7) / 8);
  const int tiles_per_wave = (int)((((U + chunks - 1) / chunks) + 7) / 8);
  a.npass = (tiles_per_wave + kTabTPW - 1) / kTabTPW;
  const size_t lds = 160 * 1024;
  static DeviceMask cap;
  {
    const int rc = raise_lds_cap(k_tables_b3, cap);
    if (rc) return rc;
  }
  hipLaunchKernelGGL(k_tables_b3, dim3(chunks, 2, parts), dim3(512), lds, stream, a);
  GNNRAG_LAUNCH_CHECK();
  return 0;
}

}

extern "C" int gnnrag_relation_tables_planes(const gnnrag_csr* csr, const void* planes, const float* ins, const float* W,
                                             float* P, int32_t D, int32_t I, gnnrag_stream_t stream) {
  if (!csr || !planes || !ins || !W || !P || D <= 0 || I <= 0 || csr->rel_total < 0) return GNNRAG_E_BADARG;
  if (csr->rel_total == 0) return 0;
  return gnnrag::tables_vq_launch(csr, planes, ins, W, P, D, I, -1, (hipStream_t)stream);
}
```

Baseline: 2.939 billion.

## Fuse next layer's softmax/pair build into tables_vq launch and add fused frontier kernel

Flattens the tables_vq grid to one dimension and appends extra blocks that run the next layer's softmax over scores and build the per-edge probability/relation pair array. This lets that work run concurrently with the relation-table GEMM instead of in a separate launch. The frontier build and table/walk kernels are also split into device functions so a fused frontier launch can reuse them. In exchange the code gains complexity, mixes heterogeneous blocks that share one LDS allocation, and adds ordering dependencies between layers.

```diff
diff --git a/gnn-rag_amd/csrc/dense_internal.h b/gnn-rag_amd/csrc/dense_internal.h
--- a/gnn-rag_amd/csrc/dense_internal.h
+++ b/gnn-rag_amd/csrc/dense_internal.h
@@ -3,8 +3,24 @@
 
 namespace gnnrag {
 
+struct VqSoftmaxJob {
+  const float* score;
+  float* dist;
+  const int32_t* rp0;
+  const int32_t* rp1;
+  const int2* em;
+  const int32_t* from;
+  const float* w0;
+  const float* w1;
+  int2* pr;
+  int64_t F;
+  int32_t N, parts, items;
+};
 int tables_vq_launch_z(const gnnrag_csr* csr, const void* planes, const float* ins, const float* W, float* P, int32_t D,
-                       int32_t I, int32_t only_dir, float* zero, int64_t zero_n, hipStream_t stream);
+                       int32_t I, int32_t only_dir, float* zero, int64_t zero_n, hipStream_t stream,
+                       const VqSoftmaxJob* softmax = nullptr);
+bool tables_vq_accepts(const gnnrag_csr* csr, const void* planes, const float* ins, const float* W, const float* P, int32_t D,
+                       int32_t I);
 
 int update_b3_launch_z(const float* h, const float* nbr, const float* W, const float* b, const float* w_s,
                        const float* b_s, const float* mask, float* h_out, float* score, int64_t BN, int32_t D,
@@ -25,6 +41,9 @@
 
 int frontier_build_z(const gnnrag_csr* csr, const float* dist, void* fws, size_t fws_bytes, float* zero_a,
                      int64_t zero_na, float* zero_b, int64_t zero_nb, hipStream_t stream);
+int frontier_fused_launch(const gnnrag_csr* csr, const float* dist, void* fws, size_t fws_bytes, float* zero_a,
+                          int64_t zero_na, float* zero_b, int64_t zero_nb, const float* T_fwd, const float* T_inv,
+                          const float* ins, const float* W, float* P, float* nbr, int32_t D, int32_t I, hipStream_t stream);
 const uint8_t* frontier_row_flags(const gnnrag_csr* csr, const void* fws);
 
 int update_score_fused_z(const float* h, const float* nbr, const float* W, const float* b, const float* w_s,
diff --git a/gnn-rag_amd/csrc/frontier.hip b/gnn-rag_amd/csrc/frontier.hip
--- a/gnn-rag_amd/csrc/frontier.hip
+++ b/gnn-rag_amd/csrc/frontier.hip
@@ -7,7 +7,7 @@
 constexpr int kFrAltSeeds = 32;
 
 struct FrontierWs {
-  size_t counts, row_flag, rows, tflag, trows, seeds, seedinfo, total;
+  size_t counts, row_flag, rows, tflag, trows, seeds, seedinfo, todo, total;
 };
 
 static FrontierWs frontier_ws(const gnnrag_csr* csr) {
@@ -23,19 +23,17 @@
   w.trows = take(RT * sizeof(int32_t));
   w.seeds = take((size_t)csr->B * kFrAltSeeds * sizeof(int32_t));
   w.seedinfo = take((size_t)2 * csr->B * sizeof(int32_t));
+  w.todo = take((size_t)2 * csr->B * sizeof(int32_t));
   w.total = off;
   return w;
 }
 
-__global__ __launch_bounds__(kFrThreads) void k_frontier_build(
+__device__ __forceinline__ void frontier_build_body(
     const float* __restrict__ dist, const int32_t* __restrict__ rp0, const int32_t* __restrict__ rp1,
     const int2* __restrict__ el0, const int2* __restrict__ el1, const int32_t* __restrict__ rel_off, int N,
-    uint8_t* __restrict__ row_flag, int32_t* __restrict__ rows, uint8_t* __restrict__ tflag,
-    int32_t* __restrict__ trows, int32_t* __restrict__ counts, int32_t* __restrict__ seeds,
-    int32_t* __restrict__ seedinfo, float* __restrict__ zero_a, long long zero_na, float* __restrict__ zero_b,
-    long long zero_nb) {
-  __shared__ int s_seed[kFrSeedCap];
-  __shared__ int s_ns, s_wsum[kFrThreads / 64];
+    uint8_t* row_flag, int32_t* rows, uint8_t* tflag, int32_t* trows, int32_t* counts, int32_t* seeds,
+    int32_t* seedinfo, float* zero_a, long long zero_na, float* zero_b, long long zero_nb, int* s_seed, int& s_ns,
+    int* s_wsum, int& nrow_out, int& ntr_out) {
   const int g = blockIdx.x, tid = threadIdx.x, lane = tid & 63, wave = tid >> 6;
   const int roff = rel_off[g], Rg = rel_off[g + 1] - roff;
   const size_t n0 = (size_t)g * N;
@@ -94,7 +92,7 @@
     }
   }
   __syncthreads();
-  auto compact = [&](const uint8_t* flag, int n, int first, int32_t* list, int32_t* count_out) {
+  auto compact = [&](const uint8_t* flag, int n, int first, int32_t* list, int32_t* count_out) -> int {
     int base = 0;
     for (int c0 = 0; c0 < n; c0 += kFrThreads) {
       const int i = c0 + tid;
@@ -113,9 +111,24 @@
       __syncthreads();
     }
     if (tid == 0) *count_out = base;
+    return base;
   };
-  compact(row_flag + n0, N, (int)n0, rows + n0, counts + 2 * g);
-  compact(tflag + roff, Rg, roff, trows + roff, counts + 2 * g + 1);
+  nrow_out = compact(row_flag + n0, N, (int)n0, rows + n0, counts + 2 * g);
+  ntr_out = compact(tflag + roff, Rg, roff, trows + roff, counts + 2 * g + 1);
+}
+
+__global__ __launch_bounds__(kFrThreads) void k_frontier_build(
+    const float* __restrict__ dist, const int32_t* __restrict__ rp0, const int32_t* __restrict__ rp1,
+    const int2* __restrict__ el0, const int2* __restrict__ el1, const int32_t* __restrict__ rel_off, int N,
+    uint8_t* __restrict__ row_flag, int32_t* __restrict__ rows, uint8_t* __restrict__ tflag,
+    int32_t* __restrict__ trows, int32_t* __restrict__ counts, int32_t* __restrict__ seeds,
+    int32_t* __restrict__ seedinfo, float* __restrict__ zero_a, long long zero_na, float* __restrict__ zero_b,
+    long long zero_nb) {
+  __shared__ int s_seed[kFrSeedCap];
+  __shared__ int s_ns, s_wsum[kFrThreads / 64];
+  int nrow, ntr;
+  frontier_build_body(dist, rp0, rp1, el0, el1, rel_off, N, row_flag, rows, tflag, trows, counts, seeds, seedinfo, zero_a,
+                      zero_na, zero_b, zero_nb, s_seed, s_ns, s_wsum, nrow, ntr);
 }
 
 struct TabFrArgs {
@@ -131,13 +144,72 @@
   int32_t dense;
 };
 
+template <int U>
+__device__ __forceinline__ void tab_fr_partial(const TabFrArgs& a, int d, int c0, int tile, int cnt, const int32_t* list,
+                                               int wave, int lane, f32x4 (&acc)[4]) {
+  const int fr = lane & 15, fg = lane >> 4;
+  const int D = a.D, K = a.I * D, ldw = (2 * a.I + 1) * D;
+  const f32x4 zero4 = {0.f, 0.f, 0.f, 0.f};
+  const int m = tile * 16 + fr;
+  const int prow = a.dense ? (m < cnt ? m : cnt - 1) : list[m < cnt ? m : cnt - 1];
+  const int2 br = a.rel_rows[prow];
+  const float* trow = a.T[d] + (size_t)br.y * D;
+  const float* qrow = a.ins + (size_t)br.x * a.I * D;
+  const float* wrow[4];
+#pragma unroll
+  for (int nt = 0; nt < 4; ++nt) wrow[nt] = a.W + (size_t)min(c0 + nt * 16 + fr, D - 1) * ldw + (size_t)(1 + d) * D;
+#pragma unroll
+  for (int nt = 0; nt < 4; ++nt) acc[nt] = zero4;
+  const int nkg = (K + 15) >> 4;
+  for (int kg0 = wave; kg0 < nkg; kg0 += 4 * U) {
+    f32x4 av[U], bv[U][4];
+#pragma unroll
+    for (int u = 0; u < U; ++u) {
+      const int k = (kg0 + 4 * u) * 16 + fg * 4;
+      av[u] = zero4;
+#pragma unroll
+      for (int nt = 0; nt < 4; ++nt) bv[u][nt] = zero4;
+      if (k < K) {
+        const int i = k / D, kk = k - i * D;
+        const f32x4 t = *reinterpret_cast<const f32x4*>(trow + kk);
+        const f32x4 q = *reinterpret_cast<const f32x4*>(qrow + (size_t)i * D + kk);
+        av[u] = __builtin_elementwise_max(t * q, zero4);
+#pragma unroll
+        for (int nt = 0; nt < 4; ++nt) bv[u][nt] = *reinterpret_cast<const f32x4*>(wrow[nt] + (size_t)2 * i * D + kk);
+      }
+    }
+#pragma unroll
+    for (int u = 0; u < U; ++u)
+#pragma unroll
+      for (int nt = 0; nt < 4; ++nt)
+#pragma unroll
+        for (int e = 0; e < 4; ++e) acc[nt] = __builtin_amdgcn_mfma_f32_16x16x4f32(av[u][e], bv[u][nt][e], acc[nt], 0, 0, 0);
+  }
+}
+
+__device__ __forceinline__ void tab_fr_store(const TabFrArgs& a, int d, int c0, int tile, int cnt, const int32_t* list,
+                                             int lane, const f32x4 (&acc)[4], float (*part)[4][64][4]) {
+  const int fr = lane & 15, fg = lane >> 4;
+  const int D = a.D;
+#pragma unroll
+  for (int nt = 0; nt < 4; ++nt) {
+    const f32x4 v = ((acc[nt] + *reinterpret_cast<const f32x4*>(&part[0][nt][lane][0])) +
+                     *reinterpret_cast<const f32x4*>(&part[1][nt][lane][0])) +
+                    *reinterpret_cast<const f32x4*>(&part[2][nt][lane][0]);
+    const int col = c0 + nt * 16 + fr;
+#pragma unroll
+    for (int rr = 0; rr < 4; ++rr) {
+      const int mm = tile * 16 + fg * 4 + rr;
+      if (mm < cnt && col < D) a.P[((size_t)d * a.rel_total + (a.dense ? mm : list[mm])) * D + col] = v[rr];
+    }
+  }
+}
+
 __global__ __launch_bounds__(256) void k_tables_frontier(TabFrArgs a, int tiles_per_q) {
   __shared__ __attribute__((aligned(16))) float s_part[3][4][64][4];
   const int lane = threadIdx.x & 63, wave = threadIdx.x >> 6;
-  const int fr = lane & 15, fg = lane >> 4;
-  const int D = a.D, K = a.I * D, ldw = (2 * a.I + 1) * D;
+  const int D = a.D;
   const int ncg = (D + 63) >> 6;
-  const f32x4 zero4 = {0.f, 0.f, 0.f, 0.f};
   const int nitem = a.dense ? ((a.rel_total + 15) >> 4) * 2 * ncg : a.B * 2 * ncg;
   for (int item = blockIdx.x; item < nitem; item += gridDim.x)
   for (int tile = a.dense ? item / (2 * ncg) : 0; tile < (a.dense ? item / (2 * ncg) + 1 : tiles_per_q); ++tile) {
@@ -149,59 +221,14 @@
     if (tile * 16 >= cnt) break;
     const int32_t* list = a.dense ? nullptr : a.list + a.rel_off[g];
     const int c0 = cg * 64;
-    const int m = tile * 16 + fr;
-    const int prow = a.dense ? (m < cnt ? m : cnt - 1) : list[m < cnt ? m : cnt - 1];
-    const int2 br = a.rel_rows[prow];
-    const float* trow = a.T[d] + (size_t)br.y * D;
-    const float* qrow = a.ins + (size_t)br.x * a.I * D;
-    const float* wrow[4];
-#pragma unroll
-    for (int nt = 0; nt < 4; ++nt) wrow[nt] = a.W + (size_t)min(c0 + nt * 16 + fr, D - 1) * ldw + (size_t)(1 + d) * D;
-    f32x4 acc[4] = {zero4, zero4, zero4, zero4};
-    const int nkg = (K + 15) >> 4;
-    for (int kg0 = wave; kg0 < nkg; kg0 += 16) {
-      f32x4 av[4], bv[4][4];
-#pragma unroll
-      for (int u = 0; u < 4; ++u) {
-        const int k = (kg0 + 4 * u) * 16 + fg * 4;
-        av[u] = zero4;
-#pragma unroll
-        for (int nt = 0; nt < 4; ++nt) bv[u][nt] = zero4;
-        if (k < K) {
-          const int i = k / D, kk = k - i * D;
-          const f32x4 t = *reinterpret_cast<const f32x4*>(trow + kk);
-          const f32x4 q = *reinterpret_cast<const f32x4*>(qrow + (size_t)i * D + kk);
-          av[u] = __builtin_elementwise_max(t * q, zero4);
-#pragma unroll
-          for (int nt = 0; nt < 4; ++nt) bv[u][nt] = *reinterpret_cast<const f32x4*>(wrow[nt] + (size_t)2 * i * D + kk);
-        }
-      }
-#pragma unroll
-      for (int u = 0; u < 4; ++u)
-#pragma unroll
-        for (int nt = 0; nt < 4; ++nt)
-#pragma unroll
-          for (int e = 0; e < 4; ++e) acc[nt] = __builtin_amdgcn_mfma_f32_16x16x4f32(av[u][e], bv[u][nt][e], acc[nt], 0, 0, 0);
-    }
+    f32x4 acc[4];
+    tab_fr_partial<4>(a, d, c0, tile, cnt, list, wave, lane, acc);
     if (wave > 0) {
 #pragma unroll
       for (int nt = 0; nt < 4; ++nt) *reinterpret_cast<f32x4*>(&s_part[wave - 1][nt][lane][0]) = acc[nt];
     }
     __syncthreads();
-    if (wave == 0) {
-#pragma unroll
-      for (int nt = 0; nt < 4; ++nt) {
-        const f32x4 v = ((acc[nt] + *reinterpret_cast<const f32x4*>(&s_part[0][nt][lane][0])) +
-                         *reinterpret_cast<const f32x4*>(&s_part[1][nt][lane][0])) +
-                        *reinterpret_cast<const f32x4*>(&s_part[2][nt][lane][0]);
-        const int col = c0 + nt * 16 + fr;
-#pragma unroll
-        for (int rr = 0; rr < 4; ++rr) {
-          const int mm = tile * 16 + fg * 4 + rr;
-          if (mm < cnt && col < D) a.P[((size_t)d * a.rel_total + (a.dense ? mm : list[mm])) * D + col] = v[rr];
-        }
-      }
-    }
+    if (wave == 0) tab_fr_store(a, d, c0, tile, cnt, list, lane, acc, s_part);
     __syncthreads();
   }
 }
@@ -230,129 +257,274 @@
 constexpr int kWfCap = kWfThreads * kWfPer;
 constexpr int kWfAltMin = 4096;
 
+__device__ __forceinline__ bool walk_fr_alt(const WalkFrArgs& a, int g, int len) {
+  return a.seedinfo[2 * g] > 0 && len > kWfAltMin && a.seedinfo[2 * g + 1] <= (len >> 2);
+}
+
+__device__ __forceinline__ f32x4 walk_fr_alt_wave(const WalkFrArgs& a, int g, int n, int roff, int Rg, int nseed, int lane) {
+  const int D = a.D;
+  const int col = 4 * lane;
+  const bool cok = col < D;
+  f32x4 acc = {0.f, 0.f, 0.f, 0.f};
+  for (int si = 0; si < nseed; ++si) {
+    const int sn = a.seeds[g * kFrAltSeeds + si];
+    const float ps = a.dist[sn];
+    const int sb = a.rp0[sn] + a.rp1[sn], se = a.rp0[sn + 1] + a.rp1[sn + 1];
+    for (int c0 = sb; c0 < se; c0 += 64) {
+      const int j = c0 + lane;
+      const int2 e = j < se ? a.edge_m[j] : make_int2(-1, 0);
+      float p = 0.f;
+      if (e.x == n) {
+        p = ps;
+        if (a.w0) {
+          const int f = a.m_from[j];
+          p *= f < a.F ? a.w0[f] : a.w1[f - a.F];
+        }
+      }
+      unsigned long long m = __ballot(p != 0.f);
+      while (m) {
+        const int l = __builtin_ctzll(m);
+        m &= m - 1;
+        const float pl = __int_as_float(__builtin_amdgcn_readlane(__float_as_int(p), l));
+        const int rm = __builtin_amdgcn_readlane(e.y, l);
+        const int dq = rm > Rg ? 1 : 0;
+        const int rl = dq ? rm - (Rg + 1) : rm;
+        if (cok) acc += pl * *reinterpret_cast<const f32x4*>(a.P + ((size_t)(1 - dq) * a.rel_total + roff + rl) * D + col);
+      }
+    }
+  }
+  return acc;
+}
+
+template <int THREADS, int PER>
+__device__ __forceinline__ void walk_fr_node(const WalkFrArgs& a, int g, int n, int roff, int Rg, int2* s_live, int* s_wsum,
+                                             float (*s_red)[256]) {
+  static_assert(THREADS * PER == kWfCap, "a pass is kWfCap records");
+  constexpr int kWaves = THREADS / 64;
+  const int tid = threadIdx.x, lane = tid & 63, wave = tid >> 6;
+  const int D = a.D;
+  const int col = 4 * lane;
+  const bool cok = col < D;
+  const f32x4 zero4 = {0.f, 0.f, 0.f, 0.f};
+  const int beg = a.rp0[n] + a.rp1[n], end = a.rp0[n + 1] + a.rp1[n + 1];
+  f32x4 acc = zero4;
+  bool split = false;
+  const int nseed = a.seedinfo[2 * g];
+  const bool alt = walk_fr_alt(a, g, end - beg);
+  if (alt && wave == 0) acc = walk_fr_alt_wave(a, g, n, roff, Rg, nseed, lane);
+  for (int c0 = beg; c0 < (alt ? beg : end); c0 += kWfCap) {
+    int2 e[PER];
+    float p[PER];
+#pragma unroll
+    for (int u = 0; u < PER; ++u) {
+      const int j = c0 + u * THREADS + tid;
+      e[u] = j < end ? a.edge_m[j] : make_int2(0, 0);
+    }
+#pragma unroll
+    for (int u = 0; u < PER; ++u) {
+      const int j = c0 + u * THREADS + tid;
+      p[u] = 0.f;
+      if (j < end) {
+        p[u] = a.dist[e[u].x];
+        if (a.w0) {
+          const int f = a.m_from[j];
+          p[u] *= f < a.F ? a.w0[f] : a.w1[f - a.F];
+        }
+      }
+    }
+    unsigned long long mk[PER];
+#pragma unroll
+    for (int u = 0; u < PER; ++u) {
+      mk[u] = __ballot(p[u] != 0.f);
+      if (lane == 0) s_wsum[u * kWaves + wave] = __popcll(mk[u]);
+    }
+    __syncthreads();
+    int nl = 0;
+#pragma unroll
+    for (int u = 0; u < PER; ++u) {
+      int off = nl;
+#pragma unroll
+      for (int w = 0; w < kWaves; ++w) {
+        const int t = s_wsum[u * kWaves + w];
+        if (w < wave) off += t;
+        nl += t;
+      }
+      if (p[u] != 0.f) {
+        const int rm = e[u].y;
+        const int d = rm > Rg ? 1 : 0;
+        const int rl = d ? rm - (Rg + 1) : rm;
+        s_live[off + __popcll(mk[u] & ((1ull << lane) - 1))] = make_int2(__float_as_int(p[u]), d * a.rel_total + roff + rl);
+      }
+    }
+    __syncthreads();
+    if (nl <= 32 && !split) {
+      if (wave == 0 && cok) {
+        for (int k = 0; k < nl; ++k) {
+          const int2 lv = s_live[k];
+          const f32x4 t = *reinterpret_cast<const f32x4*>(a.P + (size_t)lv.y * D + col);
+          acc += __int_as_float(lv.x) * t;
+        }
+      }
+    } else {
+      split = true;
+      if (cok && wave < 4) {
+        for (int k = wave; k < nl; k += 4) {
+          const int2 lv = s_live[k];
+          const f32x4 t = *reinterpret_cast<const f32x4*>(a.P + (size_t)lv.y * D + col);
+          acc += __int_as_float(lv.x) * t;
+        }
+      }
+    }
+    __syncthreads();
+  }
+  if (split) {
+    if (wave > 0 && wave < 4) *reinterpret_cast<f32x4*>(&s_red[wave - 1][col]) = acc;
+    __syncthreads();
+    if (wave == 0)
+      acc = ((acc + *reinterpret_cast<const f32x4*>(&s_red[0][col])) + *reinterpret_cast<const f32x4*>(&s_red[1][col])) +
+            *reinterpret_cast<const f32x4*>(&s_red[2][col]);
+    __syncthreads();
+  }
+  if (wave == 0 && cok) *reinterpret_cast<f32x4*>(a.out + (size_t)n * D + col) = acc;
+}
+
 __global__ __launch_bounds__(kWfThreads) void k_walk_frontier(WalkFrArgs a, int per_q) {
   __shared__ int2 s_live[kWfCap];
   __shared__ int s_wsum[kWfPer * 4];
   __shared__ __attribute__((aligned(16))) float s_red[3][256];
-  const int tid = threadIdx.x, lane = tid & 63, wave = tid >> 6;
-  const int D = a.D;
   const int g = blockIdx.x / per_q;
   const int cnt = a.counts[2 * g];
   const int roff = a.rel_off[g], Rg = a.rel_off[g + 1] - roff;
+  for (int it = blockIdx.x % per_q; it < cnt; it += per_q)
+    walk_fr_node<kWfThreads, kWfPer>(a, g, a.rows[(size_t)g * a.N + it], roff, Rg, s_live, s_wsum, s_red);
+}
+
+constexpr int kFuThreads = 1024;
+constexpr int kFuTrCap = 64;
+constexpr int kFuRowCap = 64;
+#ifndef GNNRAG_FU_TAB_UNROLL
+#define GNNRAG_FU_TAB_UNROLL 4
+#endif
+constexpr int kFuTabUnroll = GNNRAG_FU_TAB_UNROLL;
+constexpr int kFuLight = 512;
+
+__device__ __forceinline__ bool walk_fr_wave(const WalkFrArgs& a, int g, int n, int roff, int Rg, int lane) {
+  constexpr int kCh = kFuLight / 64;
+  const int D = a.D;
   const int col = 4 * lane;
   const bool cok = col < D;
-  const f32x4 zero4 = {0.f, 0.f, 0.f, 0.f};
-  for (int it = blockIdx.x % per_q; it < cnt; it += per_q) {
-    const int n = a.rows[(size_t)g * a.N + it];
-    const int beg = a.rp0[n] + a.rp1[n], end = a.rp0[n + 1] + a.rp1[n + 1];
-    f32x4 acc = zero4;
-    bool split = false;
-    const int nseed = a.seedinfo[2 * g];
-    const bool alt = nseed > 0 && end - beg > kWfAltMin && a.seedinfo[2 * g + 1] <= ((end - beg) >> 2);
-    if (alt && wave == 0) {
-      for (int si = 0; si < nseed; ++si) {
-        const int sn = a.seeds[g * kFrAltSeeds + si];
-        const float ps = a.dist[sn];
-        const int sb = a.rp0[sn] + a.rp1[sn], se = a.rp0[sn + 1] + a.rp1[sn + 1];
-        for (int c0 = sb; c0 < se; c0 += 64) {
-          const int j = c0 + lane;
-          const int2 e = j < se ? a.edge_m[j] : make_int2(-1, 0);
-          float p = 0.f;
-          if (e.x == n) {
-            p = ps;
-            if (a.w0) {
-              const int f = a.m_from[j];
-              p *= f < a.F ? a.w0[f] : a.w1[f - a.F];
-            }
-          }
-          unsigned long long m = __ballot(p != 0.f);
-          while (m) {
-            const int l = __builtin_ctzll(m);
-            m &= m - 1;
-            const float pl = __int_as_float(__builtin_amdgcn_readlane(__float_as_int(p), l));
-            const int rm = __builtin_amdgcn_readlane(e.y, l);
-            const int dq = rm > Rg ? 1 : 0;
-            const int rl = dq ? rm - (Rg + 1) : rm;
-            if (cok) acc += pl * *reinterpret_cast<const f32x4*>(a.P + ((size_t)(1 - dq) * a.rel_total + roff + rl) * D + col);
+  const int beg = a.rp0[n] + a.rp1[n], end = a.rp0[n + 1] + a.rp1[n + 1];
+  if (walk_fr_alt(a, g, end - beg)) {
+    const f32x4 acc = walk_fr_alt_wave(a, g, n, roff, Rg, a.seedinfo[2 * g], lane);
+    if (cok) *reinterpret_cast<f32x4*>(a.out + (size_t)n * D + col) = acc;
+    return true;
+  }
+  if (end - beg > kFuLight) return false;
+  int2 e[kCh];
+  float p[kCh];
+#pragma unroll
+  for (int u = 0; u < kCh; ++u) {
+    const int j = beg + u * 64 + lane;
+    e[u] = j < end ? a.edge_m[j] : make_int2(0, 0);
+  }
+  int nl = 0;
+  unsigned long long mk[kCh];
+#pragma unroll
+  for (int u = 0; u < kCh; ++u) {
+    const int j = beg + u * 64 + lane;
+    p[u] = 0.f;
+    if (j < end) {
+      p[u] = a.dist[e[u].x];
+      if (a.w0) {
+        const int f = a.m_from[j];
+        p[u] *= f < a.F ? a.w0[f] : a.w1[f - a.F];
+      }
+    }
+    mk[u] = __ballot(p[u] != 0.f);
+    nl += __popcll(mk[u]);
+  }
+  if (nl > 32) return false;
+  f32x4 acc = {0.f, 0.f, 0.f, 0.f};
+#pragma unroll
+  for (int u = 0; u < kCh; ++u) {
+    unsigned long long m = mk[u];
+    while (m) {
+      const int l = __builtin_ctzll(m);
+      m &= m - 1;
+      const float pl = __int_as_float(__builtin_amdgcn_readlane(__float_as_int(p[u]), l));
+      const int rm = __builtin_amdgcn_readlane(e[u].y, l);
+      const int d = rm > Rg ? 1 : 0;
+      const int rl = d ? rm - (Rg + 1) : rm;
+      if (cok) {
+        const f32x4 t = *reinterpret_cast<const f32x4*>(a.P + (size_t)(d * a.rel_total + roff + rl) * D + col);
+        acc += pl * t;
+      }
+    }
+  }
+  if (cok) *reinterpret_cast<f32x4*>(a.out + (size_t)n * D + col) = acc;
+  return true;
+}
+
+__global__ __launch_bounds__(kFuThreads) void k_frontier_fused(
+    const float* __restrict__ dist, const int32_t* __restrict__ rp0, const int32_t* __restrict__ rp1,
+    const int2* __restrict__ el0, const int2* __restrict__ el1, uint8_t* row_flag, uint8_t* tflag, int32_t* counts,
+    int32_t* seeds, int32_t* seedinfo, int32_t* todo, float* zero_a, long long zero_na, float* zero_b, long long zero_nb,
+    TabFrArgs ta, WalkFrArgs wa) {
+  static_assert(kFuThreads == kFrThreads, "frontier_build_body strides by kFrThreads");
+  __shared__ __attribute__((aligned(16))) float s_raw[4 * 3 * 4 * 64 * 4];
+  __shared__ int s_ns, s_wsum[2 * kFuThreads / 64], s_heavy[kFuRowCap], s_nheavy;
+  static_assert(sizeof(s_raw) >= kFrSeedCap * sizeof(int) && sizeof(s_raw) >= kWfCap * sizeof(int2) + 3 * 256 * sizeof(float),
+                "phase buffers fit");
+  const int g = blockIdx.x, tid = threadIdx.x, lane = tid & 63, wave = tid >> 6;
+  const int N = wa.N;
+  int nrow, ntr;
+  frontier_build_body(dist, rp0, rp1, el0, el1, ta.rel_off, N, row_flag, const_cast<int32_t*>(wa.rows), tflag,
+                      const_cast<int32_t*>(ta.list), counts, seeds, seedinfo, zero_a, zero_na, zero_b, zero_nb,
+                      reinterpret_cast<int*>(s_raw), s_ns, s_wsum, nrow, ntr);
+  const bool tab_here = ntr <= kFuTrCap, walk_here = tab_here && nrow <= kFuRowCap;
+  if (tid == 0) {
+    s_nheavy = 0;
+    todo[2 * g] = walk_here ? 0 : nrow;
+    todo[2 * g + 1] = tab_here ? 0 : ntr;
+  }
+  __syncthreads();
+  if (!tab_here) return;
+  const int roff = ta.rel_off[g], Rg = ta.rel_off[g + 1] - roff;
+  {
+    float (*s_part)[3][4][64][4] = reinterpret_cast<float (*)[3][4][64][4]>(s_raw);
+    const int sg = wave >> 2, w4 = wave & 3;
+    const int ncg = (ta.D + 63) >> 6;
+    const int32_t* list = ta.list + roff;
+    for (int it0 = 0; it0 < 2 * ncg; it0 += 4) {
+      const int item = it0 + sg;
+      const bool act = item < 2 * ncg;
+      const int d = item / ncg, c0 = (item - d * ncg) * 64;
+      for (int tile = 0; tile * 16 < ntr; ++tile) {
+        f32x4 acc[4];
+        if (act) {
+          tab_fr_partial<kFuTabUnroll>(ta, d, c0, tile, ntr, list, w4, lane, acc);
+          if (w4 > 0) {
+#pragma unroll
+            for (int nt = 0; nt < 4; ++nt) *reinterpret_cast<f32x4*>(&s_part[sg][w4 - 1][nt][lane][0]) = acc[nt];
           }
         }
-      }
-    }
-    for (int c0 = beg; c0 < (alt ? beg : end); c0 += kWfCap) {
-      int2 e[kWfPer];
-      float p[kWfPer];
-#pragma unroll
-      for (int u = 0; u < kWfPer; ++u) {
-        const int j = c0 + u * kWfThreads + tid;
-        e[u] = j < end ? a.edge_m[j] : make_int2(0, 0);
-      }
-#pragma unroll
-      for (int u = 0; u < kWfPer; ++u) {
-        const int j = c0 + u * kWfThreads + tid;
-        p[u] = 0.f;
-        if (j < end) {
-          p[u] = a.dist[e[u].x];
-          if (a.w0) {
-            const int f = a.m_from[j];
-            p[u] *= f < a.F ? a.w0[f] : a.w1[f - a.F];
-          }
-        }
-      }
-      unsigned long long mk[kWfPer];
-#pragma unroll
-      for (int u = 0; u < kWfPer; ++u) {
-        mk[u] = __ballot(p[u] != 0.f);
-        if (lane == 0) s_wsum[u * 4 + wave] = __popcll(mk[u]);
-      }
-      __syncthreads();
-      int nl = 0;
-#pragma unroll
-      for (int u = 0; u < kWfPer; ++u) {
-        int off = nl;
-#pragma unroll
-        for (int w = 0; w < 4; ++w) {
-          const int t = s_wsum[u * 4 + w];
-          if (w < wave) off += t;
-          nl += t;
-        }
-        if (p[u] != 0.f) {
-          const int rm = e[u].y;
-          const int d = rm > Rg ? 1 : 0;
-          const int rl = d ? rm - (Rg + 1) : rm;
-          s_live[off + __popcll(mk[u] & ((1ull << lane) - 1))] = make_int2(__float_as_int(p[u]), d * a.rel_total + roff + rl);
-        }
-      }
-      __syncthreads();
-      if (nl <= 32 && !split) {
-        if (wave == 0 && cok) {
-          for (int k = 0; k < nl; ++k) {
-            const int2 lv = s_live[k];
-            const f32x4 t = *reinterpret_cast<const f32x4*>(a.P + (size_t)lv.y * D + col);
-            acc += __int_as_float(lv.x) * t;
-          }
-        }
-      } else {
-        split = true;
-        if (cok) {
-          for (int k = wave; k < nl; k += 4) {
-            const int2 lv = s_live[k];
-            const f32x4 t = *reinterpret_cast<const f32x4*>(a.P + (size_t)lv.y * D + col);
-            acc += __int_as_float(lv.x) * t;
-          }
-        }
-      }
-      __syncthreads();
-    }
-    if (split) {
-      if (wave > 0) *reinterpret_cast<f32x4*>(&s_red[wave - 1][col]) = acc;
-      __syncthreads();
-      if (wave == 0)
-        acc = ((acc + *reinterpret_cast<const f32x4*>(&s_red[0][col])) + *reinterpret_cast<const f32x4*>(&s_red[1][col])) +
-              *reinterpret_cast<const f32x4*>(&s_red[2][col]);
-      __syncthreads();
-    }
-    if (wave == 0 && cok) *reinterpret_cast<f32x4*>(a.out + (size_t)n * D + col) = acc;
-  }
+        __syncthreads();
+        if (act && w4 == 0) tab_fr_store(ta, d, c0, tile, ntr, list, lane, acc, s_part[sg]);
+        __syncthreads();
+      }
+    }
+  }
+  if (!walk_here) return;
+  const int32_t* rows = wa.rows + (size_t)g * N;
+  for (int it = wave; it < nrow; it += kFuThreads / 64) {
+    if (!walk_fr_wave(wa, g, rows[it], roff, Rg, lane) && lane == 0) s_heavy[atomicAdd(&s_nheavy, 1)] = it;
+  }
+  __syncthreads();
+  const int nheavy = s_nheavy;
+  int2* s_live = reinterpret_cast<int2*>(s_raw);
+  float (*s_red)[256] = reinterpret_cast<float (*)[256]>(s_raw + kWfCap * 2);
+  for (int k = 0; k < nheavy; ++k)
+    walk_fr_node<kFuThreads, kWfCap / kFuThreads>(wa, g, rows[s_heavy[k]], roff, Rg, s_live, s_wsum, s_red);
 }
 
 }
@@ -398,12 +570,8 @@
   return ((((uintptr_t)a | (uintptr_t)b | (uintptr_t)c | (uintptr_t)d | (uintptr_t)e) & 15) == 0);
 }
 
-extern "C" int gnnrag_relation_tables_frontier(const gnnrag_csr* csr, const void* fws, const float* T_fwd,
-                                               const float* T_inv, const float* ins, const float* W, float* P,
-                                               int32_t D, int32_t I, gnnrag_stream_t stream) {
-  if (!csr || !fws || !T_fwd || !T_inv || !ins || !W || !P || I <= 0) return GNNRAG_E_BADARG;
-  if (!gnnrag_frontier_supported(csr, D) || !fr_aligned16(T_fwd, T_inv, ins, W, P)) return GNNRAG_E_UNSUPPORTED;
-  if (csr->rel_total == 0) return 0;
+static TabFrArgs tab_fr_args(const gnnrag_csr* csr, const void* fws, const float* T_fwd, const float* T_inv, const float* ins,
+                             const float* W, float* P, int32_t D, int32_t I, bool todo) {
   const FrontierWs w = frontier_ws(csr);
   const char* base = (const char*)fws;
   TabFrArgs a;
@@ -411,20 +579,13 @@
   a.rel_rows = (const int2*)csr->rel_rows;
   a.rel_off = csr->rel_off;
   a.list = (const int32_t*)(base + w.trows);
-  a.counts = (const int32_t*)(base + w.counts);
+  a.counts = (const int32_t*)(base + (todo ? w.todo : w.counts));
   a.P = P; a.D = D; a.I = I; a.rel_total = csr->rel_total; a.B = csr->B; a.dense = 0;
-  const int tiles_per_q = (csr->rel_max + 15) / 16;
-  const int64_t nitem = (int64_t)csr->B * 2 * ((D + 63) / 64);
-  hipLaunchKernelGGL(k_tables_frontier, dim3((unsigned)(nitem < 4096 ? nitem : 4096)), dim3(256), 0, (hipStream_t)stream, a,
-                     tiles_per_q);
-  GNNRAG_LAUNCH_CHECK();
-  return 0;
-}
-
-extern "C" int gnnrag_aggregate_fused_frontier(const gnnrag_csr* csr, const void* fws, const float* dist,
-                                               const float* P, float* out, int32_t D, gnnrag_stream_t stream) {
-  if (!csr || !fws || !dist || !P || !out) return GNNRAG_E_BADARG;
-  if (!gnnrag_frontier_supported(csr, D) || !fr_aligned16(P, out) || csr->N <= 0) return GNNRAG_E_UNSUPPORTED;
+  return a;
+}
+
+static WalkFrArgs walk_fr_args(const gnnrag_csr* csr, const void* fws, const float* dist, const float* P, float* out,
+                               int32_t D, bool todo) {
   const FrontierWs w = frontier_ws(csr);
   const char* base = (const char*)fws;
   WalkFrArgs a;
@@ -433,17 +594,74 @@
   a.w0 = csr->w_gnn[0]; a.w1 = csr->w_gnn[1];
   a.dist = dist; a.P = P; a.rel_off = csr->rel_off;
   a.rows = (const int32_t*)(base + w.rows);
-  a.counts = (const int32_t*)(base + w.counts);
+  a.counts = (const int32_t*)(base + (todo ? w.todo : w.counts));
   a.seeds = (const int32_t*)(base + w.seeds);
   a.seedinfo = (const int32_t*)(base + w.seedinfo);
   a.out = out; a.F = csr->F; a.N = csr->N; a.D = D; a.rel_total = csr->rel_total; a.B = csr->B;
+  return a;
+}
+
+static int tables_frontier_launch(const gnnrag_csr* csr, const void* fws, const float* T_fwd, const float* T_inv,
+                                  const float* ins, const float* W, float* P, int32_t D, int32_t I, bool todo,
+                                  hipStream_t stream) {
+  if (!csr || !fws || !T_fwd || !T_inv || !ins || !W || !P || I <= 0) return GNNRAG_E_BADARG;
+  if (!gnnrag_frontier_supported(csr, D) || !fr_aligned16(T_fwd, T_inv, ins, W, P)) return GNNRAG_E_UNSUPPORTED;
+  if (csr->rel_total == 0) return 0;
+  const TabFrArgs a = tab_fr_args(csr, fws, T_fwd, T_inv, ins, W, P, D, I, todo);
+  const int tiles_per_q = (csr->rel_max + 15) / 16;
+  const int64_t nitem = (int64_t)csr->B * 2 * ((D + 63) / 64);
+  hipLaunchKernelGGL(k_tables_frontier, dim3((unsigned)(nitem < 4096 ? nitem : 4096)), dim3(256), 0, stream, a, tiles_per_q);
+  GNNRAG_LAUNCH_CHECK();
+  return 0;
+}
+
+extern "C" int gnnrag_relation_tables_frontier(const gnnrag_csr* csr, const void* fws, const float* T_fwd,
+                                               const float* T_inv, const float* ins, const float* W, float* P,
+                                               int32_t D, int32_t I, gnnrag_stream_t stream) {
+  return tables_frontier_launch(csr, fws, T_fwd, T_inv, ins, W, P, D, I, false, (hipStream_t)stream);
+}
+
+static int walk_frontier_launch(const gnnrag_csr* csr, const void* fws, const float* dist, const float* P, float* out,
+                                int32_t D, bool todo, hipStream_t stream) {
+  if (!csr || !fws || !dist || !P || !out) return GNNRAG_E_BADARG;
+  if (!gnnrag_frontier_supported(csr, D) || !fr_aligned16(P, out) || csr->N <= 0) return GNNRAG_E_UNSUPPORTED;
+  const WalkFrArgs a = walk_fr_args(csr, fws, dist, P, out, D, todo);
   int per_q = 1024 / csr->B;
   if (per_q < 4) per_q = 4;
   if (per_q > 256) per_q = 256;
   if (per_q > csr->N) per_q = csr->N;
-  hipLaunchKernelGGL(k_walk_frontier, dim3((unsigned)(csr->B * per_q)), dim3(kWfThreads), 0, (hipStream_t)stream, a, per_q);
+  hipLaunchKernelGGL(k_walk_frontier, dim3((unsigned)(csr->B * per_q)), dim3(kWfThreads), 0, stream, a, per_q);
   GNNRAG_LAUNCH_CHECK();
   return 0;
+}
+
+extern "C" int gnnrag_aggregate_fused_frontier(const gnnrag_csr* csr, const void* fws, const float* dist,
+                                               const float* P, float* out, int32_t D, gnnrag_stream_t stream) {
+  return walk_frontier_launch(csr, fws, dist, P, out, D, false, (hipStream_t)stream);
+}
+
+int gnnrag::frontier_fused_launch(const gnnrag_csr* csr, const float* dist, void* fws, size_t fws_bytes, float* zero_a,
+                                  int64_t zero_na, float* zero_b, int64_t zero_nb, const float* T_fwd, const float* T_inv,
+                                  const float* ins, const float* W, float* P, float* nbr, int32_t D, int32_t I,
+                                  hipStream_t stream) {
+  if (!csr || !dist || !fws || !T_fwd || !T_inv || !ins || !W || !P || !nbr || I <= 0) return GNNRAG_E_BADARG;
+  if (!gnnrag_frontier_supported(csr, D) || !fr_aligned16(T_fwd, T_inv, ins, W, P) || !fr_aligned16(nbr) || csr->N <= 0 ||
+      csr->rel_total <= 0)
+    return GNNRAG_E_UNSUPPORTED;
+  const FrontierWs w = frontier_ws(csr);
+  if (fws_bytes < w.total) return GNNRAG_E_WORKSPACE;
+  char* base = (char*)fws;
+  const TabFrArgs ta = tab_fr_args(csr, fws, T_fwd, T_inv, ins, W, P, D, I, false);
+  const WalkFrArgs wa = walk_fr_args(csr, fws, dist, P, nbr, D, false);
+  hipLaunchKernelGGL(k_frontier_fused, dim3(csr->B), dim3(kFuThreads), 0, stream, dist, csr->row_ptr[0], csr->row_ptr[1],
+                     (const int2*)csr->edge_l[0], (const int2*)csr->edge_l[1], (uint8_t*)(base + w.row_flag),
+                     (uint8_t*)(base + w.tflag), (int32_t*)(base + w.counts), (int32_t*)(base + w.seeds),
+                     (int32_t*)(base + w.seedinfo), (int32_t*)(base + w.todo), zero_a, (long long)zero_na, zero_b,
+                     (long long)zero_nb, ta, wa);
+  GNNRAG_LAUNCH_CHECK();
+  int rc = tables_frontier_launch(csr, fws, T_fwd, T_inv, ins, W, P, D, I, true, stream);
+  if (rc) return rc;
+  return walk_frontier_launch(csr, fws, dist, P, nbr, D, true, stream);
 }
 
 extern "C" int gnnrag_frontier_read(const gnnrag_csr* csr, const void* fws, int32_t* counts2, uint8_t* row_flag_host,
diff --git a/gnn-rag_amd/csrc/softmax_layer.hip b/gnn-rag_amd/csrc/softmax_layer.hip
--- a/gnn-rag_amd/csrc/softmax_layer.hip
+++ b/gnn-rag_amd/csrc/softmax_layer.hip
@@ -234,9 +234,24 @@
   return layer_ws(csr, D, I).total;
 }
 
+static int softmax_pairs_launch(const gnnrag_csr* csr, const VqSoftmaxJob& j, gnnrag_stream_t stream) {
+  int parts = (512 + csr->B - 1) / csr->B;
+  parts = parts < 1 ? 1 : parts > 8 ? 8 : parts;
+  const size_t lds = (size_t)csr->N * sizeof(float);
+  if (csr->N <= 2048)
+    hipLaunchKernelGGL(k_softmax_pairs<2>, dim3(csr->B, parts), dim3(1024), lds, (hipStream_t)stream, j.score, j.dist, csr->N,
+                       j.rp0, j.rp1, j.em, j.from, j.w0, j.w1, j.F, j.pr);
+  else
+    hipLaunchKernelGGL(k_softmax_pairs<8>, dim3(csr->B, parts), dim3(1024), lds, (hipStream_t)stream, j.score, j.dist, csr->N,
+                       j.rp0, j.rp1, j.em, j.from, j.w0, j.w1, j.F, j.pr);
+  GNNRAG_LAUNCH_CHECK();
+  return 0;
+}
+
 static int finish_softmax(const gnnrag_csr* csr, const LayerWs& w, char* base, const float* score, float* dist_out, int32_t D,
-                          bool want_pairs, bool* pairs_done, gnnrag_stream_t stream) {
+                          bool want_pairs, bool* pairs_done, gnnrag_stream_t stream, VqSoftmaxJob* defer = nullptr) {
   if (pairs_done) *pairs_done = false;
+  if (defer) defer->score = nullptr;
   const char* env = getenv("GNNRAG_SOFTMAX_PAIRS");
   const bool enabled = !(env && env[0] == '0');
   if (want_pairs && pairs_done && enabled && csr->N <= 8192 && csr->edge_m) {
@@ -244,28 +259,33 @@
     const int rc = prior_pairs_target(csr, D, base + w.partial, w.partial_bytes, &t);
     if (rc) return rc;
     if (t.ok) {
-      int parts = (512 + csr->B - 1) / csr->B;
-      parts = parts < 1 ? 1 : parts > 8 ? 8 : parts;
-      const size_t lds = (size_t)csr->N * sizeof(float);
-      if (csr->N <= 2048)
-        hipLaunchKernelGGL(k_softmax_pairs<2>, dim3(csr->B, parts), dim3(1024), lds, (hipStream_t)stream, score, dist_out,
-                           csr->N, csr->row_ptr[0], csr->row_ptr[1], t.edge_m, t.m_from, t.w0, t.w1, t.F, t.pairs);
-      else
-        hipLaunchKernelGGL(k_softmax_pairs<8>, dim3(csr->B, parts), dim3(1024), lds, (hipStream_t)stream, score, dist_out,
-                           csr->N, csr->row_ptr[0], csr->row_ptr[1], t.edge_m, t.m_from, t.w0, t.w1, t.F, t.pairs);
-      GNNRAG_LAUNCH_CHECK();
+      VqSoftmaxJob j;
+      memset(&j, 0, sizeof(j));
+      j.score = score; j.dist = dist_out; j.rp0 = csr->row_ptr[0]; j.rp1 = csr->row_ptr[1];
+      j.em = t.edge_m; j.from = t.m_from; j.w0 = t.w0; j.w1 = t.w1; j.pr = t.pairs; j.F = t.F; j.N = csr->N;
       *pairs_done = true;
-      return 0;
+      if (defer) {
+        *defer = j;
+        return 0;
+      }
+      return softmax_pairs_launch(csr, j, stream);
     }
   }
   return gnnrag_masked_softmax(score, dist_out, csr->B, csr->N, stream);
+}
+
+static bool layer_takes_vq(const gnnrag_csr* csr, const LayerWs& w, char* base, const void* planes, const float* ins,
+                           const float* W_e2e, int32_t D, int32_t I, int32_t math) {
+  return planes && math != GNNRAG_MATH_FP32 && csr->rel_total > 0 &&
+         tables_vq_accepts(csr, planes, ins, W_e2e, (const float*)(base + w.P), D, I);
 }
 
 static int layer_body(const gnnrag_csr* csr, const LayerWs& w, char* base, const float* h, const float* dist,
                       const float* ins, const float* T_fwd, const float* T_inv, const void* planes, const float* W_e2e,
                       const float* b_e2e, const float* w_score, const float* b_score, const float* mask,
                       float* h_out, float* score_out, float* dist_out, int32_t D, int32_t I, int32_t path,
-                      int32_t math, gnnrag_stream_t stream, bool pairs_ready = false, bool* pairs_for_next = nullptr) {
+                      int32_t math, gnnrag_stream_t stream, bool pairs_ready = false, bool* pairs_for_next = nullptr,
+                      const VqSoftmaxJob* pending = nullptr, VqSoftmaxJob* defer = nullptr) {
   if (pairs_for_next) *pairs_for_next = false;
   const int64_t BN = (int64_t)csr->B * csr->N;
   int rc;
@@ -282,24 +302,34 @@
                                (uintptr_t)nbr | (uintptr_t)dist) & 15) == 0) && csr->N > 0;
     const bool frontier_form = seed_prior && only < 0 && fr_aligned && gnnrag_frontier_supported(csr, D) && csr->rel_total > 0;
     if (frontier_form) {
+      if (pending) return GNNRAG_E_BADARG;
       void* fws = base + w.fws;
       const bool gated = update_rows_supported(h, nbr, W_e2e, h_out, BN, D, I, math);
       if (!gated) GNNRAG_HIP(hipMemsetAsync(nbr, 0, (size_t)BN * D * sizeof(float), (hipStream_t)stream));
-      rc = frontier_build_z(csr, dist, fws, w.fws_bytes, score_out, BN, nbr + (size_t)BN * D, D, (hipStream_t)stream);
-      if (rc) return rc;
-      rc = gnnrag_relation_tables_frontier(csr, fws, T_fwd, T_inv, ins, W_e2e, P, D, I, stream);
-      if (rc) return rc;
-      rc = gnnrag_aggregate_fused_frontier(csr, fws, dist, P, nbr, D, stream);
-      if (rc) return rc;
+      const char* fenv = getenv("GNNRAG_FRONTIER_FUSED");
+      if (!(fenv && fenv[0] == '0')) {
+        rc = frontier_fused_launch(csr, dist, fws, w.fws_bytes, score_out, BN, nbr + (size_t)BN * D, D, T_fwd, T_inv, ins,
+                                   W_e2e, P, nbr, D, I, (hipStream_t)stream);
+        if (rc) return rc;
+      } else {
+        rc = frontier_build_z(csr, dist, fws, w.fws_bytes, score_out, BN, nbr + (size_t)BN * D, D, (hipStream_t)stream);
+        if (rc) return rc;
+        rc = gnnrag_relation_tables_frontier(csr, fws, T_fwd, T_inv, ins, W_e2e, P, D, I, stream);
+        if (rc) return rc;
+        rc = gnnrag_aggregate_fused_frontier(csr, fws, dist, P, nbr, D, stream);
+        if (rc) return rc;
+      }
       rc = update_score_fused_rows(h, nbr, gated ? frontier_row_flags(csr, fws) : nullptr, W_e2e, b_e2e, w_score, b_score,
                                    mask, h_out, score_out, BN, D, I, math, (hipStream_t)stream, true);
       if (rc) return rc;
-      return finish_softmax(csr, w, base, score_out, dist_out, D, only < 0, pairs_for_next, stream);
+      return finish_softmax(csr, w, base, score_out, dist_out, D, only < 0, pairs_for_next, stream, defer);
     }
     rc = GNNRAG_E_UNSUPPORTED;
     bool score_zeroed = false;
+    if (pending && !layer_takes_vq(csr, w, base, planes, ins, W_e2e, D, I, math)) return GNNRAG_E_BADARG;
     if (planes && math != GNNRAG_MATH_FP32 && csr->rel_total > 0) {
-      rc = tables_vq_launch_z(csr, planes, ins, W_e2e, P, D, I, one_dir ? only : -1, score_out, BN, (hipStream_t)stream);
+      rc = tables_vq_launch_z(csr, planes, ins, W_e2e, P, D, I, one_dir ? only : -1, score_out, BN, (hipStream_t)stream,
+                              pending);
       score_zeroed = rc == 0;
     }
     if (rc == GNNRAG_E_UNSUPPORTED) rc = gnnrag_relation_tables(csr, T_fwd, T_inv, ins, W_e2e, P, D, I, math, stream);
@@ -310,8 +340,9 @@
     rc = update_score_fused_z(h, nbr, W_e2e, b_e2e, w_score, b_score, mask, h_out, score_out, BN, D, I, math,
                               (hipStream_t)stream, score_zeroed);
     if (rc) return rc;
-    return finish_softmax(csr, w, base, score_out, dist_out, D, only < 0, pairs_for_next, stream);
+    return finish_softmax(csr, w, base, score_out, dist_out, D, only < 0, pairs_for_next, stream, defer);
   } else {
+    if (pending) return GNNRAG_E_BADARG;
     float* agg = (float*)(base + w.agg);
     rc = gnnrag_aggregate(csr, dist, ins, T_fwd, T_inv, agg, D, I, base + w.partial, w.partial_bytes, stream);
     if (rc) return rc;
@@ -412,6 +443,13 @@
   const float* h = h0;
   const float* dist = dist0;
   bool pairs_ready = false;
+  const char* tsenv = getenv("GNNRAG_TABLES_SOFTMAX");
+  const bool fused_path = (path & 0xf) == GNNRAG_PATH_FUSED ||
+                          ((path & 0xf) == GNNRAG_PATH_AUTO && fused_is_cheaper(csr->B, csr->N, csr->rel_total, D, I));
+  const bool ride = !(tsenv && tsenv[0] == '0') && upfront && fused_path && want_planes && planes_written &&
+                    !(path & (GNNRAG_PATH_ONLY_FWD | GNNRAG_PATH_ONLY_INV));
+  VqSoftmaxJob job;
+  memset(&job, 0, sizeof(job));
   for (int j = 0; j < L; ++j) {
     const gnnrag_layer_params& p = layers[j];
     float* hj = h_out + (size_t)j * BN * D;
@@ -426,10 +464,16 @@
     }
     if (!planes_written) planes = nullptr;
     bool pairs_next = false;
+    const VqSoftmaxJob pending = job;
+    const bool next_takes = ride && j + 1 < L &&
+                            layer_takes_vq(csr, w, base, planes_all + (size_t)(j + 1) * plane_bytes, ins, layers[j + 1].W_e2e, D, I,
+                                           math);
     const int rc = layer_body(csr, w, base, h, dist, ins, T, T + RD, planes, p.W_e2e, p.b_e2e, w_score, b_score, mask, hj, sj,
                               dj, D, I, j == 0 ? path : (path & ~GNNRAG_PATH_SEED_PRIOR), math, stream, pairs_ready,
-                              j + 1 < L ? &pairs_next : nullptr);
-    if (rc) return rc;
+                              j + 1 < L ? &pairs_next : nullptr, pending.score ? &pending : nullptr,
+                              next_takes ? &job : nullptr);
+    if (rc) return rc;
+    if (!next_takes) job.score = nullptr;
     pairs_ready = pairs_next;
     h = hj;
     dist = dj;
diff --git a/gnn-rag_amd/csrc/tables_b3.hip b/gnn-rag_amd/csrc/tables_b3.hip
--- a/gnn-rag_amd/csrc/tables_b3.hip
+++ b/gnn-rag_amd/csrc/tables_b3.hip
@@ -281,6 +281,8 @@
   int32_t dir0;
   float* zero;
   int64_t zero_n;
+  int32_t gx, ndir;
+  VqSoftmaxJob sm;
 };
 
 template <int CTN, int UN>
@@ -330,14 +332,14 @@
 }
 
 template <int CTN>
-__device__ __forceinline__ void tables_vq_part(const VqArgs& a, unsigned char* lds, int col0) {
+__device__ __forceinline__ void tables_vq_part(const VqArgs& a, unsigned char* lds, int col0, int bx, int by) {
   constexpr int RB = kTabSlots * 16;
   constexpr int PL = kTabNTH * 16 * RB;
   constexpr int NKB = kTabNKB;
   const int tid = threadIdx.x, lane = tid & 63, wave = tid >> 6;
   const int fr = lane & 15, fg = lane >> 4;
-  const int d = a.dir0 + blockIdx.y;
-  const int g = blockIdx.x / a.nchunk, ch = blockIdx.x - g * a.nchunk;
+  const int d = a.dir0 + by;
+  const int g = bx / a.nchunk, ch = bx - g * a.nchunk;
   const int D = a.D, I = a.I;
   const int r0 = a.rel_off[g], r1 = a.rel_off[g + 1];
   if (r1 <= r0) return;
@@ -451,20 +453,126 @@
   }
 }
 
+template <int ITEMS>
+__device__ __forceinline__ void vq_softmax_pairs(const VqSoftmaxJob& j, unsigned char* lds, int idx) {
+  float* s_dist = reinterpret_cast<float*>(lds);
+  float* red = s_dist + ((j.N + 3) & ~3);
+  float* bcast = red + 16;
+  const int g = idx / j.parts, part = idx - g * j.parts;
+  const int N = j.N;
+  const float* s = j.score + (size_t)g * N;
+  float* o = j.dist + (size_t)g * N;
+  const int tid = threadIdx.x, lane = tid & 63, wave = tid >> 6;
+  float v[2][ITEMS], m[2];
+#pragma unroll
+  for (int hv = 0; hv < 2; ++hv) {
+    m[hv] = -INFINITY;
+#pragma unroll
+    for (int k = 0; k < ITEMS; ++k) {
+      const int i = tid + hv * 512 + k * 1024;
+      v[hv][k] = i < N ? s[i] : -INFINITY;
+      m[hv] = fmaxf(m[hv], v[hv][k]);
+    }
+  }
+#pragma unroll
+  for (int hv = 0; hv < 2; ++hv) {
+#pragma unroll
+    for (int off = 32; off > 0; off >>= 1) m[hv] = fmaxf(m[hv], __shfl_xor(m[hv], off, 64));
+    if (lane == 0) red[wave + 8 * hv] = m[hv];
+  }
+  __syncthreads();
+  if (tid == 0) {
+    float mm = red[0];
+    for (int w = 1; w < 16; ++w) mm = fmaxf(mm, red[w]);
+    *bcast = mm;
+  }
+  __syncthreads();
+  const float mx = *bcast;
+  __syncthreads();
+  float sum[2];
+#pragma unroll
+  for (int hv = 0; hv < 2; ++hv) {
+    sum[hv] = 0.f;
+#pragma unroll
+    for (int k = 0; k < ITEMS; ++k) {
+      v[hv][k] = expf(v[hv][k] - mx);
+      sum[hv] += v[hv][k];
+    }
+  }
+#pragma unroll
+  for (int hv = 0; hv < 2; ++hv) {
+#pragma unroll
+    for (int off = 32; off > 0; off >>= 1) sum[hv] += __shfl_xor(sum[hv], off, 64);
+    if (lane == 0) red[wave + 8 * hv] = sum[hv];
+  }
+  __syncthreads();
+  if (tid == 0) {
+    float t = 0.f;
+    for (int w = 0; w < 16; ++w) t += red[w];
+    *bcast = t;
+  }
+  __syncthreads();
+  const float total = *bcast;
+#pragma unroll
+  for (int hv = 0; hv < 2; ++hv)
+#pragma unroll
+    for (int k = 0; k < ITEMS; ++k) {
+      const int i = tid + hv * 512 + k * 1024;
+      if (i < N) {
+        const float d = v[hv][k] / total;
+        s_dist[i] = d;
+        if (part == 0) o[i] = d;
+      }
+    }
+  __syncthreads();
+  const int64_t n0 = (int64_t)g * N;
+  const int64_t beg = (int64_t)j.rp0[n0] + j.rp1[n0], end = (int64_t)j.rp0[n0 + N] + j.rp1[n0 + N];
+  const int64_t lo = beg + (end - beg) * part / j.parts, hi = beg + (end - beg) * (part + 1) / j.parts;
+  typedef int i32x2 __attribute__((ext_vector_type(2)));
+  constexpr int kVqSmUnroll = 8;
+  for (int64_t j0 = lo + tid; j0 < hi; j0 += 512 * kVqSmUnroll) {
+    i32x2 e[kVqSmUnroll];
+#pragma unroll
+    for (int u = 0; u < kVqSmUnroll; ++u) {
+      const int64_t jj = j0 + u * 512;
+      e[u] = jj < hi ? __builtin_nontemporal_load(reinterpret_cast<const i32x2*>(j.em) + jj) : i32x2{0, 0};
+    }
+#pragma unroll
+    for (int u = 0; u < kVqSmUnroll; ++u) {
+      const int64_t jj = j0 + u * 512;
+      if (jj < hi) {
+        const unsigned src = (unsigned)(e[u].x - (int)n0);
+        float p = src < (unsigned)N ? s_dist[src] : 0.f;
+        if (j.w0) {
+          const int f = j.from[jj];
+          p *= f < j.F ? j.w0[f] : j.w1[f - j.F];
+        }
+        j.pr[jj] = make_int2(__float_as_int(p), e[u].y);
+      }
+    }
+  }
+}
+
 __global__ __launch_bounds__(512, 2) void k_tables_vq(VqArgs a) {
   extern __shared__ __attribute__((aligned(16))) unsigned char lds[];
+  const int ntab = a.gx * a.ndir * 2;
+  const int lin = blockIdx.x;
+  if (lin >= ntab) {
+    if (a.sm.items == 2) vq_softmax_pairs<2>(a.sm, lds, lin - ntab);
+    else vq_softmax_pairs<8>(a.sm, lds, lin - ntab);
+    return;
+  }
   if (a.zero) {
-    const int64_t nb = (int64_t)gridDim.x * gridDim.y * gridDim.z;
-    const int64_t lin = blockIdx.x + (int64_t)gridDim.x * (blockIdx.y + (int64_t)gridDim.y * blockIdx.z);
-    for (int64_t i = lin * 512 + threadIdx.x; i < a.zero_n; i += nb * 512) a.zero[i] = 0.f;
-  }
+    for (int64_t i = (int64_t)lin * 512 + threadIdx.x; i < a.zero_n; i += (int64_t)ntab * 512) a.zero[i] = 0.f;
+  }
+  const int bx = lin % a.gx, by = (lin / a.gx) % a.ndir;
   const int NT = (a.D + 15) >> 4;
-  const int h = blockIdx.z;
+  const int h = lin / (a.gx * a.ndir);
   const int ctn = h == 0 ? a.ct0 : NT - a.ct0;
   const int col0 = h == 0 ? 0 : a.ct0 * 16;
   switch (ctn) {
-    case 6: tables_vq_part<6>(a, lds, col0); break;
-    case 7: tables_vq_part<7>(a, lds, col0); break;
+    case 6: tables_vq_part<6>(a, lds, col0, bx, by); break;
+    case 7: tables_vq_part<7>(a, lds, col0, bx, by); break;
     default: break;
   }
 }
@@ -738,10 +846,16 @@
   return tables_vq_launch_z(csr, planes, ins, W, P, D, I, only_dir, nullptr, 0, stream);
 }
 
+bool tables_vq_accepts(const gnnrag_csr* csr, const void* planes, const float* ins, const float* W, const float* P, int32_t D,
+                       int32_t I) {
+  if (!tables_vq_shape_ok(D, I) || csr->rel_total < 1024) return false;
+  return (((uintptr_t)planes | (uintptr_t)ins | (uintptr_t)W | (uintptr_t)P) & 15) == 0;
+}
+
 int tables_vq_launch_z(const gnnrag_csr* csr, const void* planes, const float* ins, const float* W, float* P, int32_t D,
-                       int32_t I, int32_t only_dir, float* zero, int64_t zero_n, hipStream_t stream) {
-  if (!tables_vq_shape_ok(D, I) || csr->rel_total < 1024 || only_dir > 1) return GNNRAG_E_UNSUPPORTED;
-  if ((((uintptr_t)planes | (uintptr_t)ins | (uintptr_t)W | (uintptr_t)P) & 15) != 0) return GNNRAG_E_UNSUPPORTED;
+                       int32_t I, int32_t only_dir, float* zero, int64_t zero_n, hipStream_t stream,
+                       const VqSoftmaxJob* softmax) {
+  if (!tables_vq_accepts(csr, planes, ins, W, P, D, I) || only_dir > 1) return GNNRAG_E_UNSUPPORTED;
   VqArgs a;
   memset(&a, 0, sizeof(a));
   a.planes = (const unsigned char*)planes; a.ins = ins; a.W = W; a.P = P;
@@ -763,12 +877,23 @@
   a.nchunk = nchunk;
   a.zero = zero;
   a.zero_n = zero ? zero_n : 0;
+  a.gx = csr->B * nchunk;
+  a.ndir = ndir;
+  unsigned extra = 0;
+  if (softmax) {
+    if (softmax->N <= 0 || softmax->N > 8192 || (size_t)softmax->N * sizeof(float) + 256 > 160 * 1024) return GNNRAG_E_BADARG;
+    a.sm = *softmax;
+    a.sm.items = softmax->N <= 2048 ? 2 : 8;
+    int parts = nchunk * ndir;
+    a.sm.parts = parts < 1 ? 1 : parts > 8 ? 8 : parts;
+    extra = (unsigned)(csr->B * a.sm.parts);
+  }
   static DeviceMask cap;
   {
     const int rc = raise_lds_cap(k_tables_vq, cap);
     if (rc) return rc;
   }
-  hipLaunchKernelGGL(k_tables_vq, dim3(csr->B * nchunk, ndir, 2), dim3(512), 160 * 1024, stream, a);
+  hipLaunchKernelGGL(k_tables_vq, dim3((unsigned)(a.gx * ndir * 2) + extra), dim3(512), 160 * 1024, stream, a);
   GNNRAG_LAUNCH_CHECK();
   return 0;
 }
```

Result: slower. 2.770 billion (-5.8%).
